# GreatV/oar-ocr

Measured on AMD Instinct MI355X. Metric: images/sec end-to-end PP-OCRv6 det+rec, higher is better.
Workload: dtype f32; 1 GPU; PP-OCRv6-tiny-class det+rec (synthetic-weight graphs: det 447089 params, rec 1135700 params, V=6906), batch=32 synthetic 960x960 pages per GPU, 40 text lines/page; timed region = u8 pages in pageable HOST memory -> oar_ocr_predict -> oar_ocr_decode -> sorted boxes + texts + scores on the host; image_batch_size=32, region_batch_size=256, parallelism=image-parallel x1

## Files before the change

### oar_ocr_amd/build.py

```python
from __future__ import annotations

import os
import subprocess
import sys
from concurrent.futures import ThreadPoolExecutor
from pathlib import Path

HERE = Path(__file__).resolve().parent
CSRC = HERE / "csrc"
LIBDIR = HERE / "lib"
LIB = LIBDIR / "libOarMi355x.so"
SOURCES = ["common.cc", "onnx_parse.cc", "engine.cc", "db_host.cc", "poly_host.cc", "pipeline.cc", "c_api.cc", "ctc_host.cc", "image_decode.cc", "image_misc_decode.cc", "jpeg_decode.cc", "layout.cc", "kernels.hip", "igemm.hip", "igemm_ws_1x1.hip", "igemm_ws_gen.hip", "igemm_ws_x6.hip", "igemm_os_x6.hip", "igemm_ws3.hip", "igemm_rs3_x6.hip", "prepost.hip", "contours.hip", "jpeg.hip", "layout.hip", "dsblock.hip", "dsblock_k3s1.hip", "dsblock_k3s2.hip", "dsblock_k5s1.hip", "dsblock_k5s2.hip", "dsblock_wa_a.hip", "dsblock_wa_b.hip", "dsblock_rs_k3s11.hip", "dsblock_rs_k3s21.hip", "dsblock_rs_k3s12.hip", "dsblock_rs_k3s22.hip", "dsblock_rs_dbg.hip", "dsblock_cs.hip", "dsblock_pc.hip", "dsblock_rs2.hip", "ctc_head_x6.hip", "chain.hip", "attention_x6.hip", "igemm_lk_x6.hip"]
HIPCC = os.environ.get("HIPCC", "/opt/rocm/bin/hipcc")
FLAGS = ["--offload-arch=gfx950", "-O3", "-std=c++17", "-fPIC", "-ffp-contract=off", "-fno-fast-math",
         "-Wno-unused-result", "-Wno-pass-failed"]
if os.environ.get("OAR_DSB_ABLATIONS"):
    FLAGS.append("-DOAR_DSB_ABLATIONS")


def _stale(out: Path, deps) -> bool:
    if not out.exists():
        return True
    t = out.stat().st_mtime
    return any(Path(d).stat().st_mtime > t for d in deps)


def build_lib(force: bool = False, verbose: bool = False) -> Path:
    LIBDIR.mkdir(exist_ok=True)
    objdir = LIBDIR / "obj"
    objdir.mkdir(exist_ok=True)
    headers = list(CSRC.glob("*.h")) + list(CSRC.glob("*.inc")) + [HERE.parent / "include" / "oar_mi355x.h"]
    jobs = []
    for s in SOURCES:
        src = CSRC / s
        obj = objdir / (s.replace(".", "_") + ".o")
        if force or _stale(obj, [src] + headers):
            jobs.append((src, obj))

    def cc(job):
        src, obj = job
        cmd = [HIPCC] + FLAGS + ["-c", str(src), "-o", str(obj)]
        if verbose:
            print(" ".join(cmd), flush=True)
        r = subprocess.run(cmd, capture_output=True, text=True)
        if r.returncode != 0:
            raise RuntimeError(f"hipcc failed for {src.name}:\n{r.stderr[-4000:]}")
        return obj

    if jobs:
        with ThreadPoolExecutor(max_workers=min(8, len(jobs))) as ex:
            list(ex.map(cc, jobs))
    objs = [objdir / (s.replace(".", "_") + ".o") for s in SOURCES]
    if force or jobs or _stale(LIB, objs):
        cmd = [HIPCC, "--offload-arch=gfx950", "-shared", "-fPIC", "-o", str(LIB)] + [str(o) for o in objs] + ["-lpthread", "-lz"]
        r = subprocess.run(cmd, capture_output=True, text=True)
        if r.returncode != 0:
            raise RuntimeError(f"link failed:\n{r.stderr[-4000:]}")
    return LIB


def csrc_fingerprint() -> str:
    import hashlib
    h = hashlib.sha256()
    for f in sorted(CSRC.iterdir()):
        if f.suffix in (".hip", ".inc", ".cc", ".h"):
            h.update(f.name.encode()); h.update(f.read_bytes())
    return h.hexdigest()[:16]


if __name__ == "__main__":
    p = build_lib(force="--force" in sys.argv, verbose=True)
    print(p, p.stat().st_size)
```

### oar_ocr_amd/csrc/engine.cc

```cpp
#include "engine.h"

#include "dsblock.h"

#include <algorithm>
#include <cmath>
#include <cstring>
#include <set>
#include <sstream>

namespace oar {

using k::Act;

static int64_t numel(const std::vector<int64_t>& d) {
    int64_t n = 1;
    for (auto v : d) n *= v;
    return n;
}

Engine::Engine(const uint8_t* onnx, size_t len, int device_id, hipStream_t caller_stream) : device_(device_id) {
    int ndev = 0;
    if (hipGetDeviceCount(&ndev) != hipSuccess || ndev <= 0)
        fail(OAR_DEVICE, "no HIP device visible: libOarMi355x has no CPU fallback");
    OAR_CHECK(device_id >= 0 && device_id < ndev, OAR_DEVICE, "device_id out of range");
// ... 502 lines not shown
        const char* fe = getenv("OAR_FUSE_SE_SCALE");
        const bool fuse = !fe || atoi(fe) != 0;
        auto cons = consumers(nodes);
        std::map<std::string, int> producer;
        for (int i = 0; i < (int)nodes.size(); ++i) for (auto& o : nodes[i].out) producer[o] = i;
        std::vector<bool> dead(nodes.size(), false);
        for (int i = 0; fuse && i < (int)nodes.size(); ++i) {
            const GNode& m = nodes[i];
            if (m.op != "Mul" || m.in.size() != 2 || m.act.kind != k::ACT_NONE || !m.residual.empty() || graph_outs.count(m.out[0])) continue;
            int gi = -1;
            for (int t = 0; t < 2; ++t) { auto pit = producer.find(m.in[t]); if (pit != producer.end() && nodes[pit->second].op == "SEGate") gi = t; }
            if (gi < 0 || cons[m.out[0]].size() != 1) continue;
            GNode& c = nodes[cons[m.out[0]][0]];
            if (c.op != "Conv" || c.in.size() < 2 || c.in.size() > 3 || c.in[0] != m.out[0] || !is_init(c.in[1]) || c.ai("group", 1) != 1) continue;
            const HostTensor& w = inits_[c.in[1]];
            if (w.dims.size() != 4 || w.dims[2] != 1 || w.dims[3] != 1) continue;
            bool plain = c.as("auto_pad", "NOTSET") == "NOTSET";
            for (auto v : c.ais("strides")) plain = plain && v == 1;
            for (auto v : c.ais("pads")) plain = plain && v == 0;
            if (!plain) continue;
            c.in.resize(4);
            c.in[0] = m.in[1 - gi];
            c.in[3] = m.in[gi];
            dead[i] = true;
        }
        std::vector<GNode> keep;
        for (int i = 0; i < (int)nodes.size(); ++i) if (!dead[i]) keep.push_back(std::move(nodes[i]));
        nodes.swap(keep);
    }
    {
        const char* fe = getenv("OAR_FUSE_SE_POOL");
        const bool fuse = !fe || atoi(fe) != 0;
        std::map<std::string, int> producer;
        for (int i = 0; i < (int)nodes.size(); ++i) for (auto& o : nodes[i].out) producer[o] = i;
        std::vector<bool> dead(nodes.size(), false);
        for (int i = 0; fuse && i < (int)nodes.size(); ++i) {
            const GNode& gp = nodes[i];
            if (gp.op != "GlobalAveragePool" || gp.in.size() != 1 || graph_outs.count(gp.out[0])) continue;
            auto pit = producer.find(gp.in[0]);
            if (pit == producer.end() || pit->second > i) continue;
            GNode& d = nodes[pit->second];
            if (d.op != "Conv" || d.out.size() != 1 || d.in.size() < 2 || d.in.size() > 3 || !is_init(d.in[1]) || !d.residual.empty()) continue;
            const HostTensor& wd = inits_[d.in[1]];
            if (wd.dims.size() != 4 || wd.dims[1] != 1 || d.ai("group", 1) != wd.dims[0] || wd.dims[0] < 8) continue;
            d.out.push_back(gp.out[0]);
            dead[i] = true;
            int readers = 0, gate = -1;
            for (int j = 0; j < (int)nodes.size(); ++j) {
                if (dead[j]) continue;
                for (size_t q = 0; q < nodes[j].in.size(); ++q) if (nodes[j].in[q] == gp.out[0]) { ++readers; if (nodes[j].op == "SEGate" && q == 0) gate = j; }
                if (nodes[j].residual == gp.out[0]) ++readers;
            }
            if (readers == 1 && gate >= 0 && !graph_outs.count(gp.out[0]) && !(fe && atoi(fe) == 1)) { Attr a; a.kind = Attr::I; a.i = 1; d.attrs["gap_raw"] = a; }
        }
        std::vector<GNode> keep;
        for (int i = 0; i < (int)nodes.size(); ++i) if (!dead[i]) keep.push_back(std::move(nodes[i]));
        nodes.swap(keep);
    }
    for (int i = 0; i < (int)nodes.size(); ++i) nodes[i].id = i;
    nodes_ = std::move(nodes);
}

struct TInfo {
    std::vector<int64_t> dims;
    Layout layout = Layout::NATIVE;
    Loc loc;
    bool host_int = false;
    std::vector<int64_t> hv;
    bool host_f = false;
    std::vector<double> hd;
    const HostTensor* ht = nullptr;
    bool is_int = false;
    bool u8_stem = false;
    std::string root;
    int gap_tiles = 0, gap_hw = 0;
    size_t bytes() const { return (size_t)std::max<int64_t>(numel(dims), 1) * 4; }
};

struct Arena {
    struct Blk { size_t off, sz; };
    std::vector<Blk> free_;
    size_t top = 0;
    static size_t al(size_t n) { return (n + 255) & ~(size_t)255; }
    size_t alloc(size_t n) {
        n = al(std::max<size_t>(n, 4));
        int best = -1;
        for (int i = 0; i < (int)free_.size(); ++i)
            if (free_[i].sz >= n && (best < 0 || free_[i].sz < free_[best].sz)) best = i;
        if (best >= 0) {
            size_t off = free_[best].off;
            if (free_[best].sz == n) free_.erase(free_.begin() + best);
            else { free_[best].off += n; free_[best].sz -= n; }
            return off;
        }
        size_t off = top;
        top += n;
        return off;
    }
    void release(size_t off, size_t n) {
        n = al(std::max<size_t>(n, 4));
        free_.push_back({off, n});
        std::sort(free_.begin(), free_.end(), [](const Blk& a, const Blk& b) { return a.off < b.off; });
        std::vector<Blk> m;
        for (auto& b : free_) {
            if (!m.empty() && m.back().off + m.back().sz == b.off) m.back().sz += b.sz;
            else m.push_back(b);
        }
        if (!m.empty() && m.back().off + m.back().sz == top) { top = m.back().off; m.pop_back(); }
        free_.swap(m);
    }
};

static std::vector<int64_t> clast_phys_dims(const std::vector<int64_t>& d) {
    std::vector<int64_t> p;
    p.push_back(d[0]);
    for (size_t i = 2; i < d.size(); ++i) p.push_back(d[i]);
    p.push_back(d[1]);
    return p;
}
static std::vector<int64_t> contig_strides(const std::vector<int64_t>& d) {
    std::vector<int64_t> s(d.size(), 1);
    for (int i = (int)d.size() - 2; i >= 0; --i) s[i] = s[i + 1] * d[i + 1];
    return s;
}

struct Planner {
    Engine& E;
    Plan& P;
    std::map<std::string, TInfo> vals;
    std::map<std::string, int> last_use;
    std::map<std::string, size_t> root_bytes;
    std::map<std::string, size_t> root_off;
    Arena arena;
    int cur = 0;
    std::vector<std::pair<size_t, size_t>> temps;

    Planner(Engine& e, Plan& p) : E(e), P(p) { opset = e.opset_; }

    struct PendingResize {
        Loc xin;
        std::vector<int64_t> dims;
        int N, H, W, C, Ho, Wo, imode, ictm, inm;
        float sh, sw;
        int fh = 0, fw = 0;
    };
    std::map<std::string, PendingResize> pending_resize;
    std::map<std::string, int> sole_consumer;
    void run_resize(const PendingResize& r, Loc yl, int64_t y_off, int y_ld) {
        const PendingResize q = r;
        step([=](const RunCtx& c) { k::resize(c.s, c.at(q.xin), c.mut(yl) + y_off, q.N, q.H, q.W, q.C, q.Ho, q.Wo, q.sh, q.sw, q.imode, q.ictm, q.inm, y_ld); }, 0,
             4.0 * ((double)q.N * q.H * q.W * q.C + (double)q.N * q.Ho * q.Wo * q.C));
    }
    std::map<std::string, const GNode*> pending_convt;
    struct PendingConcat { std::vector<Loc> src; std::vector<int> c; std::vector<int64_t> dims; };
    std::map<std::string, PendingConcat> pending_concat;
    std::map<std::string, int> concat_consumer;
    void emit_concat_gather(const PendingConcat& pc, Loc yl) {
        k::ConcatGatherP gp{};
        gp.n_src = (int)pc.src.size(); gp.N = (int)pc.dims[0]; gp.Ho = (int)pc.dims[2]; gp.Wo = (int)pc.dims[3]; gp.C = (int)pc.dims[1];
        int off = 0;
        for (size_t i = 0; i < pc.src.size(); ++i) { gp.c[i] = pc.c[i]; gp.off[i] = off; gp.fh[i] = 1; gp.fw[i] = 1; off += pc.c[i]; }
        const std::vector<Loc> src = pc.src;
        step([=](const RunCtx& c) {
            k::ConcatGatherP q = gp;
            for (int i = 0; i < q.n_src; ++i) q.x[i] = c.at(src[(size_t)i]);
            k::concat_gather(c.s, q, c.mut(yl));
        }, 0, 8.0 * (double)numel(pc.dims));
    }
    void materialise_concat(const std::string& name) {
        auto it = pending_concat.find(name);
        if (it == pending_concat.end()) return;
        const PendingConcat pc = it->second;
        pending_concat.erase(it);
        vals.erase(name);
        TInfo& y = new_out(name, pc.dims, Layout::CLAST);
        emit_concat_gather(pc, y.loc);
    }
    const PendingResize* peek_pending(const std::string& name) const {
        auto it = pending_resize.find(name);
        return it == pending_resize.end() ? nullptr : &it->second;
    }
    void materialise_pending(const std::string& name) {
        auto ct = pending_convt.find(name);
        if (ct != pending_convt.end()) {
            const GNode* node = ct->second;
            pending_convt.erase(ct);
            vals.erase(name);
            op_convt(*node, false);
            return;
        }
        auto it = pending_resize.find(name);
        if (it == pending_resize.end()) return;
        const PendingResize r = it->second;
        pending_resize.erase(it);
        TInfo& y = new_out(name, r.dims, Layout::CLAST);
        run_resize(r, y.loc, 0, r.C);
    }

    TInfo& get(const std::string& name) {
        if (!pending_resize.empty() || !pending_convt.empty()) materialise_pending(name);
        if (!pending_concat.empty()) materialise_concat(name);
        auto it = vals.find(name);
        if (it != vals.end()) return it->second;
        auto ii = E.inits_.find(name);
        OAR_CHECK(ii != E.inits_.end(), OAR_MODEL_LOAD, "graph references unknown value '" + name + "'");
        TInfo t;
        t.dims = ii->second.dims;
        if (ii->second.dtype == DType::F32) {
            t.ht = &ii->second;
            t.loc.kind = Loc::CONST;
            t.loc.cptr = E.upload_const("init:" + name, ii->second.f);
        } else {
            t.host_int = true;
            t.hv = ii->second.i;
        }
        return vals[name] = t;
    }
    bool has_input(const GNode& n, size_t i) const { return i < n.in.size() && !n.in[i].empty(); }

    Loc alloc_arena(size_t bytes, const std::string& root) {
        Loc l;
        l.kind = Loc::ARENA;
        l.off = (int64_t)arena.alloc(bytes);
        P.arena_bytes = std::max(P.arena_bytes, arena.top);
        if (!root.empty()) { root_bytes[root] = bytes; root_off[root] = (size_t)l.off; }
        return l;
    }
    Loc alloc_temp(size_t bytes) {
        Loc l = alloc_arena(bytes, "");
        temps.push_back({(size_t)l.off, bytes});
        return l;
    }
    std::map<std::string, std::vector<std::string>> root_aliases;
    TInfo& new_out(const std::string& name, const std::vector<int64_t>& dims, Layout lay) {
        TInfo t;
        t.dims = dims; t.layout = lay; t.root = name;
        t.loc = alloc_arena(t.bytes(), name);
        root_aliases[name].push_back(name);
        return vals[name] = t;
    }
    void adopt_root(const std::string& out, const std::string& tmp) {
        auto it = vals.find(out);
        if (it == vals.end() || tmp.empty() || tmp == out || it->second.root != tmp) return;
        auto rb = root_bytes.find(tmp);
        if (rb != root_bytes.end()) { root_bytes[out] = rb->second; root_off[out] = root_off[tmp]; root_bytes.erase(tmp); root_off.erase(tmp); }
        std::vector<std::string> moved;
        moved.swap(root_aliases[tmp]);
        root_aliases.erase(tmp);
        std::vector<std::string>& dst = root_aliases[out];
        for (auto& a : moved) {
            auto va = vals.find(a);
            if (va != vals.end() && va->second.root == tmp) { va->second.root = out; dst.push_back(a); }
        }
        it->second.root = out;
    }
    TInfo& alias_out(const std::string& name, const TInfo& src, const std::vector<int64_t>& dims, Layout lay, int64_t byte_off = 0) {
        TInfo t;
        t.dims = dims; t.layout = lay; t.root = src.root; t.loc = src.loc; t.ht = nullptr;
        if (t.loc.kind == Loc::CONST) t.loc.cptr = (const float*)((const char*)t.loc.cptr + byte_off);
        else t.loc.off += byte_off;
        if (!t.root.empty()) root_aliases[t.root].push_back(name);
        return vals[name] = t;
    }
    void step(std::function<void(const RunCtx&)> f, double flops = 0, double bytes = 0) {
        P.steps.push_back(std::move(f));
        P.flops += flops; P.bytes += bytes; P.n_kernels++;
        step_chain.push_back(-1);
        step_node.push_back(cur);
        static const bool dbg_steps = [] { const char* e = getenv("OAR_DEBUG_STEPS"); return e && atoi(e) != 0; }();
        if (dbg_steps) {
            const GNode* g = cur >= 0 && cur < (int)E.nodes_.size() ? &E.nodes_[(size_t)cur] : nullptr;
            P.step_ops.push_back(g ? g->op + " -> " + (g->out.empty() ? std::string("?") : g->out[0]) : std::string("?"));
        }
    }

    struct ChainRec {
        k::ChainOpD d;
        Loc in, out, res;
        int64_t rows = 0;
        int64_t fix_n = 0, fix_T = 0;
        std::function<std::vector<float>()> make_w;
        const float* dev_bias = nullptr;
        const float* dev_gamma = nullptr;
        double flops = 0, bytes = 0;
        int node = 0;
        std::string out_root;
    };
    std::vector<int> step_chain;
    std::vector<int> step_node;
    std::vector<ChainRec> chain_recs;
    bool chain_on = [] { const char* e = getenv("OAR_FUSE_CHAIN"); return !e || atoi(e) != 0; }();
    static bool chain_loc_ok(const Loc& l) { return l.kind == Loc::ARENA || l.kind == Loc::INPUT || (l.kind == Loc::CONST && l.cptr); }
    static k::ChainRef chain_ref(const Loc& l) {
        k::ChainRef r;
        if (l.kind == Loc::ARENA) { r.kind = 1; r.v = (unsigned long long)l.off; }
        else if (l.kind == Loc::INPUT) { r.kind = 2; r.v = (unsigned long long)l.off; }
        else if (l.kind == Loc::CONST) { r.kind = 0; r.v = (unsigned long long)reinterpret_cast<uintptr_t>(l.cptr); }
        return r;
    }
    void step_chainable(std::function<void(const RunCtx&)> f, ChainRec rec, double flops, double bytes) {
        step(std::move(f), flops, bytes);
        if (!chain_on) return;
        rec.flops = flops; rec.bytes = bytes; rec.node = cur;
        step_chain.back() = (int)chain_recs.size();
        chain_recs.push_back(std::move(rec));
    }
    bool chain_run_open() const { return chain_on && !step_chain.empty() && step_chain.back() >= 0; }
    static std::vector<float> chain_weight_conv(const HostTensor& W) {
        const int64_t Co = W.dims[0], Ci = W.dims[1], kw = W.dims[3], K = kw * Ci;
        std::vector<float> w((size_t)Co * K);
        for (int64_t co = 0; co < Co; ++co)
            for (int64_t ci = 0; ci < Ci; ++ci)
                for (int64_t b = 0; b < kw; ++b) w[(size_t)co * K + b * Ci + ci] = W.f[(size_t)((co * Ci + ci) * kw + b)];
        return w;
    }
    static std::vector<float> chain_weight_linear(const HostTensor& B, bool transB) {
        const int64_t K = transB ? B.dims[1] : B.dims[0], N = transB ? B.dims[0] : B.dims[1];
        std::vector<float> w((size_t)N * K);
        for (int64_t kk = 0; kk < K; ++kk)
            for (int64_t nn = 0; nn < N; ++nn) w[(size_t)nn * K + kk] = transB ? B.f[(size_t)(nn * K + kk)] : B.f[(size_t)(kk * N + nn)];
// ... 336 lines not shown
                float r1 = x - fh;
                std::memcpy(&um, &r1, 4); um &= 0xFFFF0000u;
                float fm; std::memcpy(&fm, &um, 4);
                float r2 = r1 - fm;
                std::memcpy(&ul, &r2, 4); ul &= 0xFFFF0000u;
                int64_t nf = r / 16, c = r % 16, kp = k / 32, half = (k % 32) / 16, g = (k % 16) / 4, e = half * 4 + k % 4;
                size_t lane = (size_t)(c + 16 * g);
                size_t base = (size_t)((nf * KP + kp) * 3) * 64 * 8;
                f[base + (0 * 64 + lane) * 8 + e] = (uint16_t)(uh >> 16);
                f[base + (1 * 64 + lane) * 8 + e] = (uint16_t)(um >> 16);
                f[base + (2 * 64 + lane) * 8 + e] = (uint16_t)(ul >> 16);
            }
        std::vector<float> out(f.size() / 2);
        std::memcpy(out.data(), f.data(), f.size() * 2);
        return out;
    }
    static std::vector<float> to_fragments(int fmt, const std::vector<float>& w, int64_t rows, int64_t K) {
        if (fmt == k::IGEMM_W_X6RS) return to_fragment_x6_rs(w, rows, K);
        return fmt == k::IGEMM_W_X6 ? to_fragment_x6(w, rows, K) : to_fragment_order(w, rows, K);
    }
    const float* conv_weight_igemm(const GNode& n, const HostTensor& W, int fmt) {
        std::string key = "igemm" + std::to_string(fmt) + ":" + n.in[1];
        auto it = E.dev_consts_.find(key);
        if (it != E.dev_consts_.end()) return it->second;
        int64_t Co = W.dims[0], Ci = W.dims[1], kh = W.dims[2], kw = W.dims[3];
        int64_t K = kh * kw * Ci, Cp = (Co + 63) / 64 * 64;
        std::vector<float> w((size_t)Cp * K, 0.f);
        for (int64_t co = 0; co < Co; ++co)
            for (int64_t ci = 0; ci < Ci; ++ci)
                for (int64_t a = 0; a < kh; ++a)
                    for (int64_t b = 0; b < kw; ++b)
                        w[(size_t)co * K + (a * kw + b) * Ci + ci] = W.f[((co * Ci + ci) * kh + a) * kw + b];
        (void)Cp;
        w.resize((size_t)Co * K);
        return E.upload_const(key, to_fragments(fmt, w, Co, K));
    }
    const float* conv_weight_cs(const GNode& dwn, const GNode& pwn, const HostTensor& WD, const HostTensor& WP, const std::vector<float>* bias_dw, const std::vector<float>* bias_pw) {
        std::string key = "dscs:" + dwn.in[1] + ":" + pwn.in[1];
        auto it = E.dev_consts_.find(key);
        if (it != E.dev_consts_.end()) return it->second;
        const int64_t C = WD.dims[0], ks = WD.dims[2], Co = WP.dims[0], nch = C / 16, nft = Co / 16;
        const size_t blk = k::dsblock_cs_block_bytes((int)ks, (int)nft), dwb = (size_t)(((ks * ks + 1) * 64 + 1023) / 1024 * 1024);
        std::vector<float> out(blk * (size_t)nch / 4 + (size_t)Co, 0.f);
        if (bias_pw) std::copy(bias_pw->begin(), bias_pw->begin() + Co, out.begin() + (ptrdiff_t)(blk * (size_t)nch / 4));
        auto split = [](float x, uint16_t& h, uint16_t& m, uint16_t& l) {
            uint32_t u, um, ul;
            std::memcpy(&u, &x, 4);
            const uint32_t uh = u & 0xFFFF0000u;
            float fh; std::memcpy(&fh, &uh, 4);
            const float r1 = x - fh;
            std::memcpy(&um, &r1, 4); um &= 0xFFFF0000u;
            float fm; std::memcpy(&fm, &um, 4);
            const float r2 = r1 - fm;
            std::memcpy(&ul, &r2, 4);
            h = (uint16_t)(uh >> 16); m = (uint16_t)(um >> 16); l = (uint16_t)(ul >> 16);
        };
        for (int64_t c = 0; c < nch; ++c) {
            char* b = reinterpret_cast<char*>(out.data()) + (size_t)c * blk;
            float* dw = reinterpret_cast<float*>(b);
            for (int64_t t = 0; t <= ks * ks; ++t)
                for (int64_t q = 0; q < 16; ++q) {
                    const int64_t ch = c * 16 + q;
                    dw[t * 16 + q] = t < ks * ks ? WD.f[(size_t)(ch * ks * ks + t)] : (bias_dw ? (*bias_dw)[(size_t)ch] : 0.f);
                }
            for (int64_t f = 0; f < nft; ++f) {
                uint16_t* lh = reinterpret_cast<uint16_t*>(b + dwb + (size_t)f * 1536);
                uint16_t* md = reinterpret_cast<uint16_t*>(b + dwb + (size_t)f * 1536 + 1024);
                for (int64_t g = 0; g < 4; ++g)
                    for (int64_t m = 0; m < 16; ++m)
                        for (int64_t e = 0; e < 4; ++e) {
                            uint16_t h, mm, l;
                            split(WP.f[(size_t)((f * 16 + m) * C + c * 16 + g * 4 + e)], h, mm, l);
                            const size_t lane = (size_t)(g * 16 + m);
                            lh[lane * 8 + e] = l; lh[lane * 8 + 4 + e] = h; md[lane * 4 + e] = mm;
                        }
            }
        }
        return E.upload_const(key, out);
    }
    const float* conv_weight_dw(const GNode& n, const HostTensor& W) {
        std::string key = "dw:" + n.in[1];
        auto it = E.dev_consts_.find(key);
        if (it != E.dev_consts_.end()) return it->second;
        int64_t C = W.dims[0], kh = W.dims[2], kw = W.dims[3];
        std::vector<float> w((size_t)C * kh * kw);
        for (int64_t c = 0; c < C; ++c)
            for (int64_t a = 0; a < kh; ++a)
                for (int64_t b = 0; b < kw; ++b) w[(size_t)(a * kw + b) * C + c] = W.f[(c * kh + a) * kw + b];
        return E.upload_const(key, w);
    }
    const float* conv_weight_direct(const GNode& n, const HostTensor& W) {
        std::string key = "direct:" + n.in[1];
        auto it = E.dev_consts_.find(key);
        if (it != E.dev_consts_.end()) return it->second;
        int64_t Co = W.dims[0], cpg = W.dims[1], kh = W.dims[2], kw = W.dims[3];
        std::vector<float> w((size_t)Co * cpg * kh * kw);
        for (int64_t co = 0; co < Co; ++co)
            for (int64_t ci = 0; ci < cpg; ++ci)
                for (int64_t a = 0; a < kh; ++a)
                    for (int64_t b = 0; b < kw; ++b)
                        w[(size_t)(((a * kw + b) * cpg + ci) * Co + co)] = W.f[((co * cpg + ci) * kh + a) * kw + b];
        return E.upload_const(key, w);
    }
    const float* convt_weight(const GNode& n, const HostTensor& W, bool igemm, int fmt = 0) {
        std::string key = (igemm ? "convt_ig" + std::to_string(fmt) + ":" : std::string("convt_dir:")) + n.in[1];
        auto it = E.dev_consts_.find(key);
        if (it != E.dev_consts_.end()) return it->second;
        int64_t Ci = W.dims[0], Co = W.dims[1], kh = W.dims[2], kw = W.dims[3];
        std::vector<float> w;
        if (igemm) {
            int64_t rows = kh * kw * Co;
            w.assign((size_t)rows * Ci, 0.f);
            for (int64_t ci = 0; ci < Ci; ++ci)
                for (int64_t co = 0; co < Co; ++co)
                    for (int64_t a = 0; a < kh; ++a)
                        for (int64_t b = 0; b < kw; ++b)
                            w[(size_t)((a * kw + b) * Co + co) * Ci + ci] = W.f[((ci * Co + co) * kh + a) * kw + b];
            w = to_fragments(fmt, w, rows, Ci);
        } else {
            w.assign((size_t)kh * kw * Ci * Co, 0.f);
            for (int64_t ci = 0; ci < Ci; ++ci)
                for (int64_t co = 0; co < Co; ++co)
                    for (int64_t a = 0; a < kh; ++a)
                        for (int64_t b = 0; b < kw; ++b)
                            w[(size_t)(((a * kw + b) * Ci + ci) * Co + co)] = W.f[((ci * Co + co) * kh + a) * kw + b];
        }
        return E.upload_const(key, w);
    }
    const float* linear_weight(const std::string& name, const HostTensor& B, bool transB, int fmt) {
        std::string key = "lin" + std::to_string(fmt) + ":" + (transB ? "t:" : "") + name;
        auto it = E.dev_consts_.find(key);
        if (it != E.dev_consts_.end()) return it->second;
        int64_t K = transB ? B.dims[1] : B.dims[0], N = transB ? B.dims[0] : B.dims[1];
        std::vector<float> w((size_t)N * K, 0.f);
        for (int64_t kk = 0; kk < K; ++kk)
            for (int64_t nn = 0; nn < N; ++nn) w[(size_t)nn * K + kk] = transB ? B.f[nn * K + kk] : B.f[kk * N + nn];
        return E.upload_const(key, to_fragments(fmt, w, N, K));
    }

    void get_pads(const GNode& n, int64_t H, int64_t W, int64_t kh, int64_t kw, int64_t sh, int64_t sw, int64_t dh, int64_t dw,
                  int64_t& pt, int64_t& pl, int64_t& pb, int64_t& pr) {
        std::vector<int64_t> pads = n.ais("pads");
        pt = pl = pb = pr = 0;
        if (pads.size() == 4) { pt = pads[0]; pl = pads[1]; pb = pads[2]; pr = pads[3]; }
        std::string ap = n.as("auto_pad", "NOTSET");
        if (ap == "SAME_UPPER" || ap == "SAME_LOWER") {
            int64_t oh = (H + sh - 1) / sh, ow = (W + sw - 1) / sw;
            int64_t th = std::max<int64_t>((oh - 1) * sh + (kh - 1) * dh + 1 - H, 0), tw = std::max<int64_t>((ow - 1) * sw + (kw - 1) * dw + 1 - W, 0);
            if (ap == "SAME_UPPER") { pt = th / 2; pb = th - pt; pl = tw / 2; pr = tw - pl; }
            else { pb = th / 2; pt = th - pb; pr = tw / 2; pl = tw - pr; }
        }
    }

    void op_conv(const GNode& n) {
        if (n.in.size() > 3 && !n.in[3].empty()) {
            TInfo xg = get(n.in[0]), gt = get(n.in[3]);
            const TInfo& wg = get(n.in[1]);
            bool ok = xg.dims.size() == 4 && !xg.host_int && !gt.host_int && wg.ht && wg.ht->dims.size() == 4 && gt.loc.kind != Loc::NONE && n.residual.empty();
            if (ok) {
                const int64_t N = xg.dims[0], C = xg.dims[1], HW = xg.dims[2] * xg.dims[3];
                ok = numel(gt.dims) == N * C && gt.dims.size() >= 2 && gt.dims[0] == N && gt.dims[1] == C && wg.ht->dims[1] == C && C % 8 == 0 &&
                     k::conv_igemm_se_ok(N * HW, (int)C, (int)wg.ht->dims[0], (int)HW);
            }
            if (!ok) {
                GNode mul;
                mul.op = "Mul"; mul.in = {n.in[0], n.in[3]}; mul.out = {n.out[0] + "::se"};
                op_binary(mul, 2);
                GNode c2 = n;
                c2.in.resize(3);
                c2.in[0] = mul.out[0];
                op_conv(c2);
                return;
            }
        }
        PendingConcat msrc;
        {
            auto pit = pending_concat.find(n.in[0]);
            if (pit != pending_concat.end()) {
                auto wi = E.inits_.find(n.in.size() > 1 ? n.in[1] : std::string());
                const std::vector<int64_t>& pd = pit->second.dims;
                const bool still_ok = wi != E.inits_.end() && wi->second.dims.size() == 4 && wi->second.dims[2] == 1 && wi->second.dims[3] == 1 && n.residual.empty() &&
                                      !(n.in.size() > 3 && !n.in[3].empty()) && n.out.size() == 1 &&
                                      k::conv_msrc_ok((long)(pd[0] * pd[2] * pd[3]), (int)pd[1], (int)wi->second.dims[0]);
                if (getenv("OAR_DEBUG_CONCAT")) fprintf(stderr, "  conv %s reads pending concat: still_ok=%d (w4=%d res=%d gate=%d nout=%zu)\n", n.out[0].c_str(), (int)still_ok, (int)(wi != E.inits_.end() && wi->second.dims.size() == 4), (int)!n.residual.empty(), (int)(n.in.size() > 3 && !n.in[3].empty()), n.out.size());
                if (still_ok) { msrc = pit->second; TInfo keep = vals[n.in[0]]; pending_concat.erase(pit); vals[n.in[0]] = keep; }
            }
        }
        TInfo x = get(n.in[0]);
        OAR_CHECK(x.dims.size() == 4, OAR_UNSUPPORTED_OP, "Conv: only 2-D convolutions are supported");
        const TInfo& wt = get(n.in[1]);
        OAR_CHECK(wt.ht, OAR_UNSUPPORTED_OP, "Conv: weights must be an initializer");
        const HostTensor& W = *wt.ht;
        OAR_CHECK(W.dims.size() == 4 && W.dims[0] > 0 && W.dims[1] > 0 && W.dims[2] > 0 && W.dims[3] > 0, OAR_MODEL_LOAD, "Conv: weight must be rank 4 with positive dims at " + n.out[0]);
        int64_t N = x.dims[0], Cin = x.dims[1], H = x.dims[2], Wd = x.dims[3];
        int64_t Cout = W.dims[0], kh = W.dims[2], kw = W.dims[3], g = n.ai("group", 1);
        OAR_CHECK(g >= 1 && W.dims[1] * g == Cin && Cout % g == 0, OAR_SHAPE_MISMATCH, "Conv: weight/input channel mismatch at " + n.out[0]);
        if (has_input(n, 2)) { const TInfo& bt = get(n.in[2]); OAR_CHECK(bt.ht && (int64_t)bt.ht->f.size() == Cout, OAR_MODEL_LOAD, "Conv: bias must be an f32 initializer of Cout elements at " + n.out[0]); }
        auto st = n.ais("strides"), dl = n.ais("dilations");
        int64_t sh = st.size() == 2 ? st[0] : 1, sw = st.size() == 2 ? st[1] : 1;
        int64_t dh = dl.size() == 2 ? dl[0] : 1, dw = dl.size() == 2 ? dl[1] : 1;
        int64_t pt, pl, pb, pr;
        get_pads(n, H, Wd, kh, kw, sh, sw, dh, dw, pt, pl, pb, pr);
        int64_t Ho = (H + pt + pb - dh * (kh - 1) - 1) / sh + 1, Wo = (Wd + pl + pr - dw * (kw - 1) - 1) / sw + 1;
        if (x.u8_stem) {
            OAR_CHECK(g == 1 && Cin == 3 && kh * kw * 3 <= 128 && n.residual.empty(), OAR_INTERNAL, "run_stem on a graph whose first node is not an RGB stem");
            const float* sb = has_input(n, 2) ? get(n.in[2]).loc.cptr : nullptr;
            TInfo& ys = new_out(n.out[0], {N, Cout, Ho, Wo}, Layout::CLAST);
            k::ConvP sp{};
            sp.N = (int)N; sp.H = (int)H; sp.W = (int)Wd; sp.Cin = 3; sp.Ho = (int)Ho; sp.Wo = (int)Wo; sp.Cout = (int)Cout;
            sp.kh = (int)kh; sp.kw = (int)kw; sp.sh = (int)sh; sp.sw = (int)sw; sp.pt = (int)pt; sp.pl = (int)pl; sp.dh = (int)dh; sp.dw = (int)dw;
            sp.groups = 1; sp.act = n.act; sp.bias = sb; sp.y_ld = (int)Cout; sp.convt2x2 = 0;
            sp.w = conv_weight_direct(n, W);
            const Loc ysl = ys.loc;
            step([=](const RunCtx& c) {
                OAR_CHECK(c.stem != nullptr, OAR_INTERNAL, "stem plan run without pages");
                k::ConvP q = sp;
                q.y = c.mut(ysl);
                k::conv_smallcin_u8(c.s, q, *c.stem);
            }, 2.0 * N * Ho * Wo * Cout * 3 * kh * kw, 3.0 * N * H * Wd + 4.0 * N * Ho * Wo * Cout);
            return;
        }
        Loc xin = msrc.src.empty() ? to_clast_loc(x) : Loc();
        const float* bias = has_input(n, 2) ? get(n.in[2]).loc.cptr : nullptr;
        Loc res;
        int res_up = 0;
        if (!n.residual.empty()) {
            const char* up_env = getenv("OAR_FUSE_RES_UP");
            const bool up_on = !up_env || atoi(up_env) != 0;
            if (const PendingResize* pr = peek_pending(n.residual)) {
                const bool f32_tile = g == 1 && Cin % 4 == 0 && Cout % 4 == 0 &&
                                      k::igemm_weight_format((long)(N * Ho * Wo), (int)(kh * kw * Cin), (int)Cout, kh == 1 && kw == 1 && sh == 1 && sw == 1 && pt == 0 && pl == 0, (int)Cin) == k::IGEMM_W_K16;
                if (up_on && f32_tile && pr->fh > 1 && pr->fh == pr->fw && pr->N == N && pr->C == Cout && pr->Ho == Ho && pr->Wo == Wo && Ho % pr->fh == 0 && Wo % pr->fw == 0 &&
                    pr->H * pr->fh == Ho && pr->W * pr->fw == Wo && N * Ho * Wo < ((int64_t)1 << 31)) {
                    res = pr->xin;
                    res_up = pr->fh;
                    pending_resize.erase(n.residual);
                }
            }
        }
        if (!n.residual.empty() && res_up == 0) {
            TInfo r = get(n.residual);
            if (r.host_int || r.dims != std::vector<int64_t>{N, Cout, Ho, Wo}) {
                GNode pre = n;
                pre.residual.clear();
                pre.out[0] = n.out[0] + "::pre";
                op_conv(pre);
                GNode add;
                add.op = "Add"; add.in = {pre.out[0], n.residual}; add.out = {n.out[0]};
                op_binary(add, 0);
                return;
            }
            res = to_clast_loc(r);
        }
        TInfo& y = new_out(n.out[0], {N, Cout, Ho, Wo}, Layout::CLAST);
        k::ConvP p{};
        p.N = (int)N; p.H = (int)H; p.W = (int)Wd; p.Cin = (int)Cin; p.Ho = (int)Ho; p.Wo = (int)Wo; p.Cout = (int)Cout;
        p.kh = (int)kh; p.kw = (int)kw; p.sh = (int)sh; p.sw = (int)sw; p.pt = (int)pt; p.pl = (int)pl; p.dh = (int)dh; p.dw = (int)dw;
        p.groups = (int)g; p.act = n.act; p.bias = bias; p.y_ld = (int)Cout; p.convt2x2 = 0; p.res_up = res_up;
        int kind;
        const int64_t cg = Cin / g, og = Cout / g;
        const char* gx_env = getenv("OAR_GROUPED_X6");
        const bool grouped_x6 = g > 1 && g < Cin && cg % 8 == 0 && og % 4 == 0 && !(n.in.size() > 3 && !n.in[3].empty()) && res_up == 0 && !(gx_env && gx_env[0] == '0') &&
                                k::conv_grouped_x6_ok((long)(N * Ho * Wo), (int)(kh * kw * cg), (int)og, (int)cg);
        std::vector<const float*> wgrp;
        std::vector<int> slices3;
        if (grouped_x6) {
            kind = 3;
            p.w_fmt = k::IGEMM_W_X6;
            const size_t per = (size_t)(og * cg * kh * kw);
            for (int64_t gi = 0; gi < g; ++gi) {
                HostTensor Wg;
                Wg.dtype = DType::F32; Wg.dims = {og, cg, kh, kw};
                Wg.f.assign(W.f.begin() + (ptrdiff_t)(gi * per), W.f.begin() + (ptrdiff_t)((gi + 1) * per));
                GNode gn = n;
                gn.in[1] = n.in[1] + "::group" + std::to_string(gi);
                wgrp.push_back(conv_weight_igemm(gn, Wg, k::IGEMM_W_X6));
            }
        }
        else if (g == 1 && Cout <= 16 && Cin > 64 && kh == 3 && kw == 3 && sh == 1 && sw == 1 && pt == 1 && pl == 1 && dh == 1 && dw == 1 && Ho == H && Wo == Wd && n.residual.empty() &&
                 !(n.in.size() > 3 && !n.in[3].empty()) && !(slices3 = k::conv3x3_n16_slices((long)(N * Ho * Wo), (int)Cin, (int)Cout, (long)(H * Wd), (int)(4 * Cout))).empty()) {
            kind = 4;
            p.w_fmt = k::IGEMM_W_X6;
            int64_t c0 = 0;
            for (int cs : slices3) {
                HostTensor Ws;
                Ws.dtype = DType::F32; Ws.dims = {Cout, (int64_t)cs, kh, kw};
                Ws.f.resize((size_t)(Cout * cs * 9));
                for (int64_t co = 0; co < Cout; ++co)
                    for (int64_t ci = 0; ci < cs; ++ci)
                        for (int64_t t = 0; t < 9; ++t) Ws.f[(size_t)((co * cs + ci) * 9 + t)] = W.f[(size_t)((co * Cin + c0 + ci) * 9 + t)];
                GNode gn = n;
                gn.in[1] = n.in[1] + "::slice" + std::to_string(c0);
                wgrp.push_back(conv_weight_igemm(gn, Ws, k::IGEMM_W_X6));
                c0 += cs;
            }
        }
        else if (g == 1 && Cin % 4 == 0) {
            kind = 0;
            const bool is1x1 = kh == 1 && kw == 1 && sh == 1 && sw == 1 && pt == 0 && pl == 0;
            const bool same3x3 = kh == 3 && kw == 3 && sh == 1 && sw == 1 && pt == 1 && pl == 1 && dh == 1 && dw == 1 && Ho == H && Wo == Wd && n.residual.empty();
            const bool lk_ok = !(n.in.size() > 3 && !n.in[3].empty()) && res_up == 0 &&
                               k::conv_lk_x6_eligible((int)kh, (int)kw, (int)sh, (int)sw, (int)pt, (int)pl, (int)dh, (int)dw, (int)H, (int)Wd, (int)Ho, (int)Wo, (int)Cin, (int)Cout, (int)(4 * Cout), (long)(N * Ho * Wo));
            p.w_fmt = k::igemm_weight_format((long)(N * Ho * Wo), (int)(kh * kw * Cin), (int)Cout, is1x1, (int)Cin, same3x3 ? (long)(H * Wd) : 0, lk_ok);
            p.w = conv_weight_igemm(n, W, p.w_fmt);
        }
        else if (g == Cin && g == Cout && Cout % 4 == 0) { kind = 1; p.w = conv_weight_dw(n, W); }
        else { kind = 2; p.w = conv_weight_direct(n, W); }
        Loc yl = y.loc;
        bool has_res = res.kind != Loc::NONE;
        Loc gate;
        if (n.in.size() > 3 && !n.in[3].empty()) {
            OAR_CHECK(kind == 0 && (p.w_fmt == k::IGEMM_W_X6 || p.w_fmt == k::IGEMM_W_K16), OAR_INTERNAL, "Conv: gate on a layer that is on neither gated kernel");
            gate = get(n.in[3]).loc;
        }
        const bool has_gate = gate.kind != Loc::NONE;
        double flops = 2.0 * N * Ho * Wo * Cout * (Cin / g) * kh * kw;
        double bytes = 4.0 * (N * H * Wd * Cin + N * Ho * Wo * Cout * (has_res ? 2 : 1) + numel(W.dims));
        if (n.out.size() > 1) {
            const int tiles = kind == 1 ? k::conv_dw_gap_tiles(p) : 0;
            if (tiles > 0 && Cout <= 1024 && n.ai("gap_raw", 0) != 0) {
                TInfo& gy = new_out(n.out[1], {N, (int64_t)tiles * Cout, 1, 1}, Layout::CLAST);
                gy.gap_tiles = tiles; gy.gap_hw = (int)(Ho * Wo);
                const Loc part = gy.loc;
                step([=](const RunCtx& c) {
                    k::ConvP q = p;
                    q.x = c.at(xin); q.y = c.mut(yl); q.residual = has_res ? c.at(res) : nullptr; q.gap_part = c.mut(part);
                    k::conv_dw(c.s, q);
                }, flops, bytes + 4.0 * N * tiles * Cout);
                return;
            }
            if (tiles > 0 && Cout <= 1024) {
                TInfo& gy = new_out(n.out[1], {N, Cout, 1, 1}, Layout::CLAST);
                const Loc gl = gy.loc, part = alloc_temp((size_t)N * tiles * Cout * sizeof(float));
                const int hw = (int)(Ho * Wo);
                step([=](const RunCtx& c) {
                    k::ConvP q = p;
                    q.x = c.at(xin); q.y = c.mut(yl); q.residual = has_res ? c.at(res) : nullptr; q.gap_part = c.mut(part);
                    k::conv_dw(c.s, q);
                }, flops, bytes + 4.0 * N * tiles * Cout);
                step([=](const RunCtx& c) { k::global_avgpool_finish(c.s, c.at(part), c.mut(gl), (int)N, tiles, (int)Cout, hw); }, 0, 4.0 * N * tiles * Cout);
                return;
            }
        }
        const bool from_concat = !msrc.src.empty();
        OAR_CHECK(!from_concat || (kind == 0 && p.w_fmt == k::IGEMM_W_X6), OAR_INTERNAL, "Conv: deferred concat in front of a layer that is not on the bf16x6 kernels");
        auto run = [=](const RunCtx& c) {
            k::ConvP q = p;
            q.y = c.mut(yl); q.residual = has_res ? c.at(res) : nullptr; q.se = has_gate ? c.at(gate) : nullptr;
            if (from_concat) {
                q.x = nullptr; q.n_msrc = (int)msrc.src.size();
                for (int i = 0; i < q.n_msrc; ++i) { q.msrc[i] = c.at(msrc.src[(size_t)i]); q.msrc_c[i] = msrc.c[(size_t)i]; }
            } else {
                q.x = c.at(xin);
            }
            if (kind == 3) {
                const int ng = p.groups, cgi = p.Cin / ng, ogi = p.Cout / ng;
                for (int gi = 0; gi < ng; ++gi) {
                    k::ConvP r = q;
                    r.groups = 1; r.Cin = cgi; r.Cout = ogi; r.x_ld = p.Cin;
                    r.x = q.x + (size_t)gi * cgi; r.y = q.y + (size_t)gi * ogi; r.w = wgrp[(size_t)gi];
                    r.bias = q.bias ? q.bias + (size_t)gi * ogi : nullptr;
                    r.residual = q.residual ? q.residual + (size_t)gi * ogi : nullptr;
                    k::conv_igemm(c.s, r);
                }
                return;
            }
            if (kind == 4) {
                int c0 = 0;
                for (size_t i = 0; i < slices3.size(); ++i) {
                    k::ConvP r = q;
                    r.Cin = slices3[i]; r.x_ld = p.Cin; r.x = q.x + c0; r.w = wgrp[i]; r.accum = i > 0 ? 1 : 0;
                    if (i > 0) r.bias = nullptr;
                    if (i + 1 < slices3.size()) r.act = k::Act{};
                    k::conv_igemm(c.s, r);
                    c0 += slices3[i];
                }
                return;
            }
            if (kind == 0) k::conv_igemm(c.s, q);
            else if (kind == 1) k::conv_dw(c.s, q);
            else k::conv_direct(c.s, q);
        };
        auto pool_after = [&]() {
            if (n.out.size() < 2) return;
            GNode gp;
            gp.op = "GlobalAveragePool"; gp.in = {n.out[0]}; gp.out = {n.out[1]};
            op_gap(gp);
        };
        if (kind == 0 && !has_gate && H == 1 && Ho == 1 && kh == 1 && pt == 0 && pb == 0 && sw == 1 && dw == 1 && Wo == Wd && Cin % 16 == 0 && Cout % 16 == 0 && k::chain_act_ok(n.act.kind) &&
            chain_loc_ok(xin) && (!has_res || chain_loc_ok(res))) {
            ChainRec r;
            r.d.type = k::CH_GEMM; r.d.K = (int)(kw * Cin); r.d.N = (int)Cout; r.d.cin = (int)Cin; r.d.pad = (int)pl;
            r.d.in_ld = (int)Cin; r.d.out_ld = (int)Cout; r.d.res_ld = (int)Cout;
            r.d.act = n.act.kind; r.d.alpha = n.act.alpha; r.d.beta = n.act.beta; r.dev_bias = bias;
            r.in = xin; r.out = yl; if (has_res) r.res = res;
            r.rows = N * Wd; r.out_root = n.out[0];
            if (kw > 1) { r.fix_n = N; r.fix_T = Wd; }
            const HostTensor* Wp = &W;
            r.make_w = [Wp]() { return chain_weight_conv(*Wp); };
            step_chainable(run, std::move(r), flops, bytes);
            pool_after();
            return;
        }
        step(run, flops, bytes);
        pool_after();
    }

    bool dsblock_shape(const GNode& n, int64_t N, int64_t C, int64_t H, int64_t W, k::DsBlockP& p) {
        const TInfo &wdt = get(n.in[1]), &wpt = get(n.in[3]);
        if (!wdt.ht || !wpt.ht) return false;
        const HostTensor &WD = *wdt.ht, &WP = *wpt.ht;
        const int64_t ks = WD.dims[2], Cout = WP.dims[0];
        if (WD.dims[0] != C || WP.dims[1] != C) return false;
        auto st = n.ais("strides");
        const int64_t sh = st.size() == 2 ? st[0] : 1, sw = st.size() == 2 ? st[1] : 1;
        int64_t pt, pl, pb, pr;
        get_pads(n, H, W, ks, ks, sh, sw, 1, 1, pt, pl, pb, pr);
        const int64_t Ho = (H + pt + pb - (ks - 1) - 1) / sh + 1, Wo = (W + pl + pr - (ks - 1) - 1) / sw + 1;
        p = k::DsBlockP{};
        p.N = (int)N; p.H = (int)H; p.W = (int)W; p.C = (int)C; p.Ho = (int)Ho; p.Wo = (int)Wo; p.Cout = (int)Cout;
        p.ks = (int)ks; p.sh = (int)sh; p.sw = (int)sw; p.pt = (int)pt; p.pl = (int)pl;
        p.act1.kind = (int)n.ai("act1", 0); p.act1.alpha = n.af("act1_alpha", 0.f); p.act1.beta = n.af("act1_beta", 0.f);
        p.act2 = n.act; p.y_ld = (int)Cout;
        p.has_res = !n.residual.empty();
        return Ho > 0 && Wo > 0;
    }
    bool dsblock_link_ok(int i) {
        if (i + 1 >= (int)E.nodes_.size()) return false;
        const GNode &n = E.nodes_[i], &m = E.nodes_[i + 1];
        if (n.op != "DSBlock" || m.op != "DSBlock" || !n.residual.empty() || !m.residual.empty() || m.in.empty() || m.in[0] != n.out[0]) return false;
        for (auto& o : E.output_names_) if (o == n.out[0]) return false;
        for (int j = 0; j < (int)E.nodes_.size(); ++j) {
            if (j == i + 1) continue;
            const GNode& q = E.nodes_[j];
            for (auto& s : q.in) if (s == n.out[0]) return false;
            if (q.residual == n.out[0]) return false;
        }
        for (size_t k = 1; k < m.in.size(); ++k) if (m.in[k] == n.out[0]) return false;
        return true;
    }
    std::map<int, bool> dsblock_pair_plan;
    void plan_dsblock_run(int first, const TInfo& x) {
        std::vector<k::DsBlockP> ps;
        std::vector<bool> link;
        int64_t N = x.dims[0], C = x.dims[1], H = x.dims[2], W = x.dims[3];
        for (int i = first; i < (int)E.nodes_.size(); ++i) {
            const GNode& q = E.nodes_[i];
            k::DsBlockP p;
            if (q.op != "DSBlock" || q.in.size() < 5 || !dsblock_shape(q, N, C, H, W, p)) break;
            ps.push_back(p);
            C = p.Cout; H = p.Ho; W = p.Wo;
            const bool ok = dsblock_link_ok(i);
            link.push_back(ok);
            if (!ok) break;
        }
        const int R = (int)ps.size();
        std::vector<double> w(std::max(R - 1, 0), -1.0);
        for (int j = 0; j + 1 < R; ++j)
            if (link[j] && k::dsblock2_eligible(ps[j], ps[j + 1])) w[j] = (double)N * ps[j].Cout * ps[j].Ho * ps[j].Wo;
        static const bool greedy_first = [] { const char* e = getenv("OAR_DSBLOCK_RS2_FIRST"); return e && atoi(e) != 0; }();
        std::vector<bool> take(std::max(R - 1, 0), false);
        if (greedy_first) {
            for (int j = 0; j + 1 < R; ++j) if (w[j] > 0) { take[j] = true; ++j; }
        } else {
            std::vector<double> best(R + 1, 0.0);
            for (int j = R - 2; j >= 0; --j) best[j] = std::max(best[j + 1], w[j] > 0 ? w[j] + best[std::min(j + 2, R)] : 0.0);
            for (int j = 0; j + 1 < R;) {
                if (w[j] > 0 && w[j] + best[std::min(j + 2, R)] >= best[j + 1]) { take[j] = true; j += 2; }
                else ++j;
            }
        }
        for (int j = 0; j < R; ++j) dsblock_pair_plan[first + j] = j + 1 < R && take[j];
    }
    bool try_dsblock_pair(const GNode& n, const TInfo& x) {
        if (cur + 1 >= (int)E.nodes_.size() || !n.residual.empty() || x.dims.size() != 4 || x.host_int) return false;
        if (!dsblock_pair_plan.count(cur)) plan_dsblock_run(cur, x);
        if (!dsblock_pair_plan[cur]) return false;
        const GNode& m = E.nodes_[cur + 1];
        k::DsBlockP pa, pb;
        const int64_t N = x.dims[0], C = x.dims[1], H = x.dims[2], W = x.dims[3];
        if (!dsblock_shape(n, N, C, H, W, pa) || !dsblock_shape(m, N, pa.Cout, pa.Ho, pa.Wo, pb) || !k::dsblock2_eligible(pa, pb)) return false;
        auto weights = [&](const GNode& d, k::DsBlockP& p) {
            const HostTensor &WD = *get(d.in[1]).ht, &WP = *get(d.in[3]).ht;
            GNode dwn, pwn;
            dwn.op = "Conv"; dwn.in = {d.in[0], d.in[1]};
            pwn.op = "Conv"; pwn.in = {d.out[0] + "::dw", d.in[3]};
            if (!d.in[2].empty()) OAR_CHECK((int64_t)get(d.in[2]).ht->f.size() == p.C, OAR_MODEL_LOAD, "DSBlock: depthwise bias size");
            if (!d.in[4].empty()) OAR_CHECK((int64_t)get(d.in[4]).ht->f.size() == p.Cout, OAR_MODEL_LOAD, "DSBlock: pointwise bias size");
            p.wd = conv_weight_dw(dwn, WD);
            p.bd = d.in[2].empty() ? nullptr : get(d.in[2]).loc.cptr;
            p.wp = conv_weight_igemm(pwn, WP, k::IGEMM_W_X6RS);
            p.bp = d.in[4].empty() ? nullptr : get(d.in[4]).loc.cptr;
        };
        weights(n, pa);
        weights(m, pb);
        Loc xin = to_clast_loc(x);
        TInfo& y = new_out(m.out[0], {N, (int64_t)pb.Cout, (int64_t)pb.Ho, (int64_t)pb.Wo}, Layout::CLAST);
        Loc yl = y.loc;
        const double px = (double)N * H * W;
        const double flops = 2.0 * px * (pa.C * (9.0 + pa.Cout) + pb.C * (9.0 + pb.Cout));
        const double bytes = 4.0 * px * (pa.C + pb.Cout);
        step([=](const RunCtx& c) {
            k::DsBlockP qa = pa, qb = pb;
            qa.x = c.at(xin); qb.y = c.mut(yl);
// ... 691 lines not shown
        Loc xin = x.loc;
        TInfo& y = new_out(n.out[0], od, clast ? Layout::CLAST : Layout::NATIVE);
        Loc yl = y.loc;
        step([=](const RunCtx& c) { k::pad_nd(c.s, c.at(xin), c.mut(yl), r, pin.data(), pout.data(), pbef.data(), imode, value); }, 0, 8.0 * numel(od));
    }

    void op_gap(const GNode& n) {
        TInfo x = get(n.in[0]);
        OAR_CHECK(x.dims.size() == 4, OAR_UNSUPPORTED_OP, "GlobalAveragePool: rank-4 only");
        Loc xin = to_clast_loc(x);
        int64_t N = x.dims[0], C = x.dims[1], HW = x.dims[2] * x.dims[3];
        TInfo& y = new_out(n.out[0], {N, C, 1, 1}, Layout::CLAST);
        Loc yl = y.loc;
        const int splits = k::global_avgpool_splits((int)N, (int)HW, (int)C);
        Loc part;
        if (splits > 1) part = alloc_temp((size_t)N * splits * C * sizeof(float));
        step([=](const RunCtx& c) { k::global_avgpool(c.s, c.at(xin), c.mut(yl), (int)N, (int)HW, (int)C, splits > 1 ? c.mut(part) : nullptr); }, 0, 4.0 * numel(x.dims));
    }

    void op_pool(const GNode& n, bool is_max) {
        TInfo x = get(n.in[0]);
        OAR_CHECK(x.dims.size() == 4, OAR_UNSUPPORTED_OP, "Pool: rank-4 only");
        auto ks = n.ais("kernel_shape"), st = n.ais("strides");
        OAR_CHECK(ks.size() == 2, OAR_UNSUPPORTED_OP, "Pool: kernel_shape");
        int64_t kh = ks[0], kw = ks[1], sh = st.size() == 2 ? st[0] : 1, sw = st.size() == 2 ? st[1] : 1;
        int64_t pt, pl, pb, pr;
        get_pads(n, x.dims[2], x.dims[3], kh, kw, sh, sw, 1, 1, pt, pl, pb, pr);
        bool ceil_mode = n.ai("ceil_mode", 0) != 0;
        auto od = [&](int64_t in, int64_t k_, int64_t s_, int64_t p0, int64_t p1) {
            int64_t t = in + p0 + p1 - k_;
            int64_t o = (ceil_mode ? (t + s_ - 1) / s_ : t / s_) + 1;
            if (ceil_mode && (o - 1) * s_ >= in + p0) --o;
            return o;
        };
        int64_t Ho = od(x.dims[2], kh, sh, pt, pb), Wo = od(x.dims[3], kw, sw, pl, pr);
        Loc xin = to_clast_loc(x);
        TInfo& y = new_out(n.out[0], {x.dims[0], x.dims[1], Ho, Wo}, Layout::CLAST);
        k::PoolP p{};
        p.N = (int)x.dims[0]; p.H = (int)x.dims[2]; p.W = (int)x.dims[3]; p.C = (int)x.dims[1]; p.Ho = (int)Ho; p.Wo = (int)Wo;
        p.kh = (int)kh; p.kw = (int)kw; p.sh = (int)sh; p.sw = (int)sw; p.pt = (int)pt; p.pl = (int)pl; p.pb = (int)pb; p.pr = (int)pr;
        p.is_max = is_max; p.count_include_pad = (int)n.ai("count_include_pad", 0);
        Loc yl = y.loc;
        auto run = [=](const RunCtx& c) { k::PoolP q = p; q.x = c.at(xin); q.y = c.mut(yl); k::pool2d(c.s, q); };
        const double bytes = 4.0 * (numel(x.dims) + numel(y.dims));
        const char* cpe = getenv("OAR_CHAIN_POOL");
        if (!(cpe && cpe[0] == '0') && !is_max && !ceil_mode && Ho == 1 && kh == x.dims[2] && kw == sw && kw * Wo <= x.dims[3] && x.dims[3] - kw * Wo < kw && pt == 0 && pl == 0 && pb == 0 && pr == 0 &&
            (p.C & 3) == 0 && kh * kw <= 64 && chain_loc_ok(xin)) {
            ChainRec r;
            r.d.type = k::CH_POOL; r.d.K = (int)kh; r.d.cin = (int)kw; r.d.pad = (int)x.dims[3]; r.d.N = p.C; r.d.in_ld = p.C; r.d.out_ld = p.C;
            r.in = xin; r.out = yl; r.rows = x.dims[0] * Wo; r.fix_n = x.dims[0]; r.fix_T = Wo; r.out_root = n.out[0];
            step_chainable(run, std::move(r), 0, bytes);
        } else {
            step(run, 0, bytes);
        }
    }

    void op_resize(const GNode& n) {
        TInfo x = get(n.in[0]);
        OAR_CHECK(x.dims.size() == 4, OAR_UNSUPPORTED_OP, "Resize: rank-4 only");
        int64_t H = x.dims[2], W = x.dims[3], Ho, Wo;
        float sh, sw;
        if (has_input(n, 3)) {
            const TInfo& sz = get(n.in[3]);
            OAR_CHECK(sz.host_int && sz.hv.size() == 4, OAR_UNSUPPORTED_OP, "Resize: sizes must be a host int tensor");
            Ho = sz.hv[2]; Wo = sz.hv[3]; sh = (float)Ho / (float)H; sw = (float)Wo / (float)W;
        } else {
            OAR_CHECK(has_input(n, 2), OAR_UNSUPPORTED_OP, "Resize: neither scales nor sizes");
            const TInfo& sc = get(n.in[2]);
            std::vector<double> scv = host_values(sc);
            OAR_CHECK(host_evaluable(sc) && scv.size() == 4, OAR_UNSUPPORTED_OP, "Resize: scales must be 4 floats known at plan time");
            sh = (float)scv[2]; sw = (float)scv[3];
            Ho = (int64_t)std::floor((float)H * sh); Wo = (int64_t)std::floor((float)W * sw);
        }
        std::string mode = n.as("mode", "nearest"), ctm = n.as("coordinate_transformation_mode", "half_pixel"), nm = n.as("nearest_mode", "round_prefer_floor");
        int imode = mode == "nearest" ? 0 : 1;
        OAR_CHECK(mode == "nearest" || mode == "linear", OAR_UNSUPPORTED_OP, "Resize: mode " + mode);
        int ictm = ctm == "asymmetric" ? 0 : ctm == "half_pixel" ? 1 : ctm == "align_corners" ? 2 : ctm == "pytorch_half_pixel" ? 3 : -1;
        OAR_CHECK(ictm >= 0, OAR_UNSUPPORTED_OP, "Resize: coordinate_transformation_mode " + ctm);
        int inm = nm == "floor" ? 0 : nm == "round_prefer_floor" ? 1 : nm == "round_prefer_ceil" ? 2 : 3;
        static const bool defer_on = [] { const char* e = getenv("OAR_DEFER_RESIZE"); return !e || atoi(e) != 0; }();
        if (defer_on && imode == 0 && x.layout == Layout::CLAST && sole_consumer.count(n.out[0])) {
            PendingResize r;
            r.xin = x.loc; r.dims = {x.dims[0], x.dims[1], Ho, Wo};
            r.N = (int)x.dims[0]; r.H = (int)H; r.W = (int)W; r.C = (int)x.dims[1]; r.Ho = (int)Ho; r.Wo = (int)Wo;
            r.imode = imode; r.ictm = ictm; r.inm = inm; r.sh = sh; r.sw = sw;
            auto factor = [&](int in, int out, float scale) {
                if (in <= 0 || out % in != 0) return 0;
                const int f = out / in;
                for (int o = 0; o < out; ++o) if (k::resize_nearest_index(o, scale, in, out, ictm, inm) != o / f) return 0;
                return f;
            };
            r.fh = factor(r.H, r.Ho, sh); r.fw = factor(r.W, r.Wo, sw);
            if (!r.fh || !r.fw) r.fh = r.fw = 0;
            pending_resize[n.out[0]] = r;
            TInfo t;
            t.dims = r.dims; t.layout = Layout::CLAST; t.root = "";
            vals[n.out[0]] = t;
            return;
        }
        Loc xin = to_clast_loc(x);
        TInfo& y = new_out(n.out[0], {x.dims[0], x.dims[1], Ho, Wo}, Layout::CLAST);
        Loc yl = y.loc;
        int N = (int)x.dims[0], C = (int)x.dims[1];
        step([=](const RunCtx& c) { k::resize(c.s, c.at(xin), c.mut(yl), N, (int)H, (int)W, C, (int)Ho, (int)Wo, sh, sw, imode, ictm, inm, C); }, 0,
             4.0 * (numel(x.dims) + numel(y.dims)));
    }

    void op_concat(const GNode& n) {
        bool absorb = false;
        if (!pending_resize.empty()) {
            int64_t axis0 = n.ai("axis", 0);
            bool ok = true, any = false;
            int64_t total_c = 0;
            for (auto& s : n.in) {
                const PendingResize* pr = peek_pending(s);
                any = any || pr;
                auto it = vals.find(s);
                if (it == vals.end() || it->second.dims.size() != 4 || it->second.layout != Layout::CLAST || it->second.host_int) { ok = false; break; }
                if ((it->second.dims[1] & 3) != 0) ok = false;
                total_c += it->second.dims[1];
            }
            absorb = any && ok && (axis0 == 1 || axis0 == -3) && (total_c & 3) == 0;
            if (!absorb) for (auto& s : n.in) materialise_pending(s);
        }
        std::vector<TInfo> xs;
        for (auto& s : n.in) { auto it = vals.find(s); xs.push_back(absorb && peek_pending(s) ? it->second : get(s)); }
        bool all_host = true, any_host = false, any_f = false;
        for (auto& t : xs) { all_host = all_host && host_evaluable(t) && t.dims.size() <= 1; any_host = any_host || t.host_int; any_f = any_f || float_like(t); }
        if (all_host && any_host) {
            std::vector<double> v;
            for (auto& t : xs) { std::vector<double> e = host_values(t); v.insert(v.end(), e.begin(), e.end()); }
            set_host(n.out[0], {(int64_t)v.size()}, v, any_f);
            return;
        }
        int r = (int)xs[0].dims.size();
        int64_t axis = n.ai("axis", 0);
        if (axis < 0) axis += r;
        bool clast = false;
        for (auto& t : xs) clast = clast || (t.layout == Layout::CLAST);
        std::vector<int64_t> od = xs[0].dims;
        od[axis] = 0;
        for (auto& t : xs) od[axis] += t.dims[axis];
        if (clast && r >= 3) {
            int pax = axis == 0 ? 0 : (axis == 1 ? r - 1 : (int)axis - 1);
            std::vector<int64_t> pod = clast_phys_dims(od);
            int64_t outer = 1, inner = 1;
            for (int i = 0; i < pax; ++i) outer *= pod[i];
            for (int i = pax + 1; i < r; ++i) inner *= pod[i];
            std::vector<Loc> ins;
            for (size_t i = 0; i < xs.size(); ++i) ins.push_back(absorb && peek_pending(n.in[i]) ? Loc() : to_clast_loc(xs[i]));
            int64_t coff = 0, total = pod[pax] * inner;
            bool plain = !absorb && r == 4 && inner == 1 && xs.size() >= 3 && (od[1] & 3) == 0;
            for (auto& t : xs) plain = plain && t.dims.size() == 4 && (t.dims[1] & 3) == 0;
            static const bool defer_on = [] { const char* e = getenv("OAR_CONCAT_DEFER"); return !(e && e[0] == '0'); }();
            if (getenv("OAR_DEBUG_CONCAT")) fprintf(stderr, "concat %s: plain=%d absorb=%d r=%d inner=%ld n=%zu consumer=%d\n", n.out[0].c_str(), (int)plain, (int)absorb, r, (long)inner, xs.size(), concat_consumer.count(n.out[0]) ? concat_consumer[n.out[0]] : -1);
            if (plain && defer_on && xs.size() <= 8 && concat_consumer.count(n.out[0])) {
                const GNode& cn = E.nodes_[concat_consumer[n.out[0]]];
                auto wi = E.inits_.find(cn.in.size() > 1 ? cn.in[1] : std::string());
                auto attr_ok = [&](const char* a, int64_t want) { auto v = cn.ais(a); for (auto e : v) if (e != want) return false; return true; };
                bool ok = wi != E.inits_.end() && wi->second.dims.size() == 4 && wi->second.dims[2] == 1 && wi->second.dims[3] == 1 && wi->second.dims[1] == od[1] && cn.ai("group", 1) == 1 &&
                          attr_ok("strides", 1) && attr_ok("pads", 0) && attr_ok("dilations", 1) && cn.residual.empty() && !(cn.in.size() > 3 && !cn.in[3].empty()) &&
                          cn.as("auto_pad", "NOTSET") == "NOTSET";
                for (auto& t : xs) ok = ok && t.layout == Layout::CLAST && (t.dims[1] & 7) == 0 && t.dims[0] == od[0] && t.dims[2] == od[2] && t.dims[3] == od[3] && !t.host_int;
                if (getenv("OAR_DEBUG_CONCAT")) {
                    fprintf(stderr, "  ok before msrc check = %d (K=%ld N=%ld) res=%d gate=%d autopad=%s\n", (int)ok, (long)od[1], wi != E.inits_.end() ? (long)wi->second.dims[0] : -1L, (int)!cn.residual.empty(), (int)(cn.in.size() > 3 && !cn.in[3].empty()), cn.as("auto_pad", "NOTSET").c_str());
                    for (auto& t : xs) fprintf(stderr, "    src layout=%d C=%ld host=%d\n", (int)(t.layout == Layout::CLAST), (long)t.dims[1], (int)t.host_int);
                }
                ok = ok && k::conv_msrc_ok((long)(od[0] * od[2] * od[3]), (int)od[1], (int)wi->second.dims[0]) && (wi->second.dims[0] & 3) == 0;
                if (ok) {
                    PendingConcat pc;
                    for (size_t i = 0; i < xs.size(); ++i) { pc.src.push_back(ins[i]); pc.c.push_back((int)xs[i].dims[1]); }
                    pc.dims = od;
                    TInfo t;
                    t.dims = od; t.layout = Layout::CLAST;
                    vals[n.out[0]] = t;
                    pending_concat[n.out[0]] = std::move(pc);
                    return;
                }
            }
            TInfo& y = new_out(n.out[0], od, Layout::CLAST);
            Loc yl = y.loc;
            if ((absorb || plain) && r == 4 && inner == 1 && xs.size() <= 8) {
                static const bool gather_on = [] { const char* e = getenv("OAR_CONCAT_GATHER"); return !(e && e[0] == '0'); }();
                bool ok = gather_on;
                for (size_t i = 0; ok && i < xs.size(); ++i) {
                    const PendingResize* pr = peek_pending(n.in[i]);
                    if (pr) ok = pr->fh > 0 && pr->fw > 0 && pr->imode == 0 && pr->Ho == od[2] && pr->Wo == od[3] && pr->H * pr->fh == pr->Ho && pr->W * pr->fw == pr->Wo && pr->N == od[0];
                    else ok = xs[i].dims[0] == od[0] && xs[i].dims[2] == od[2] && xs[i].dims[3] == od[3];
                }
                if (ok) {
                    k::ConcatGatherP gp{};
                    std::vector<Loc> src(xs.size());
                    gp.n_src = (int)xs.size(); gp.N = (int)od[0]; gp.Ho = (int)od[2]; gp.Wo = (int)od[3]; gp.C = (int)od[1];
                    double bytes = 4.0 * (double)numel(od);
                    for (size_t i = 0; i < xs.size(); ++i) {
                        const PendingResize* pr = peek_pending(n.in[i]);
                        src[i] = pr ? pr->xin : ins[i];
                        gp.c[i] = (int)xs[i].dims[1]; gp.off[i] = (int)coff; gp.fh[i] = pr ? pr->fh : 1; gp.fw[i] = pr ? pr->fw : 1;
                        bytes += 4.0 * (double)numel(xs[i].dims) / (gp.fh[i] * gp.fw[i]);
                        coff += xs[i].dims[1];
                    }
                    for (auto& nm : n.in) pending_resize.erase(nm);
                    step([=](const RunCtx& c) {
                        k::ConcatGatherP q = gp;
                        for (int i = 0; i < q.n_src; ++i) q.x[i] = c.at(src[(size_t)i]);
                        k::concat_gather(c.s, q, c.mut(yl));
                    }, 0, bytes);
                    return;
                }
            }
            for (size_t i = 0; i < xs.size(); ++i) {
                int64_t w = xs[i].dims[axis] * inner;
                Loc il = ins[i];
                int64_t off = coff;
                if (absorb && peek_pending(n.in[i])) {
                    run_resize(*peek_pending(n.in[i]), yl, off, (int)total);
                    pending_resize.erase(n.in[i]);
                } else {
                    concat_copy_step(il, yl, off, outer, w, total, n.out[0]);
                }
                coff += w;
            }
            return;
        }
        int64_t outer = 1, inner = 1;
        for (int i = 0; i < axis; ++i) outer *= od[i];
        for (int i = (int)axis + 1; i < r; ++i) inner *= od[i];
        std::vector<Loc> ins;
        for (auto& t : xs) ins.push_back(to_native_loc(t));
        TInfo& y = new_out(n.out[0], od, Layout::NATIVE);
        Loc yl = y.loc;
        int64_t coff = 0, total = od[axis] * inner;
        for (size_t i = 0; i < xs.size(); ++i) {
            int64_t w = xs[i].dims[axis] * inner;
            Loc il = ins[i];
            int64_t off = coff;
            concat_copy_step(il, yl, off, outer, w, total, n.out[0]);
            coff += w;
        }
    }
    void concat_copy_step(Loc il, Loc yl, int64_t off, int64_t outer, int64_t w, int64_t total, const std::string& out_name) {
        auto run = [=](const RunCtx& c) { k::copy2d(c.s, c.at(il), c.mut(yl) + off, outer, (int)w, (int)w, (int)total); };
        if ((w & 3) == 0 && (total & 3) == 0 && (off & 3) == 0 && chain_loc_ok(il) && yl.kind == Loc::ARENA) {
            ChainRec r;
            r.d.type = k::CH_COPY; r.d.N = (int)w; r.d.in_ld = (int)w; r.d.out_ld = (int)total;
            r.in = il; r.out = yl; r.out.off += off * 4; r.rows = outer; r.out_root = out_name;
            step_chainable(run, std::move(r), 0, 8.0 * outer * w);
        } else {
            step(run, 0, 8.0 * outer * w);
        }
    }

    void view_native(const GNode& n, const TInfo& x, const std::vector<int64_t>& od) {
        OAR_CHECK(numel(od) == numel(x.dims), OAR_SHAPE_MISMATCH, "reshape: element count mismatch at " + n.out[0]);
        if (x.layout == Layout::CLAST) {
            int r = (int)x.dims.size();
            int64_t sp = 1;
            for (int i = 2; i < r; ++i) sp *= x.dims[i];
            if (od.size() >= 3 && od[0] == x.dims[0] && od[1] == x.dims[1] && !x.ht) { alias_out(n.out[0], x, od, Layout::CLAST); return; }
            if (x.dims[1] != 1 && sp != 1) {
                TInfo& y = new_out(n.out[0], od, Layout::NATIVE);
                to_native_loc(x, y.loc);
                return;
            }
        }
        alias_out(n.out[0], x, od, Layout::NATIVE);
    }

    void op_reshape(const GNode& n) {
        TInfo x = get(n.in[0]);
        const TInfo& sh = get(n.in[1]);
        OAR_CHECK(sh.host_int, OAR_UNSUPPORTED_OP, "Reshape: shape must be known on the host");
        if (x.host_int) { TInfo o = x; o.dims.assign(sh.hv.begin(), sh.hv.end()); vals[n.out[0]] = o; return; }
        std::vector<int64_t> od(sh.hv.size());
        int64_t known = 1; int infer = -1;
        for (size_t i = 0; i < od.size(); ++i) {
            int64_t v = sh.hv[i];
            if (v == 0 && n.ai("allowzero", 0) == 0) v = x.dims[i];
            if (v == -1) { infer = (int)i; v = 1; }
            od[i] = v; known *= v;
        }
        if (infer >= 0) od[infer] = numel(x.dims) / std::max<int64_t>(known, 1);
        view_native(n, x, od);
    }

    void op_flatten(const GNode& n) {
        TInfo x = get(n.in[0]);
        int64_t ax = n.ai("axis", 1);
        if (ax < 0) ax += (int64_t)x.dims.size();
        int64_t a = 1, b = 1;
        for (int i = 0; i < (int)x.dims.size(); ++i) (i < ax ? a : b) *= x.dims[i];
        view_native(n, x, {a, b});
    }

    std::vector<int64_t> axes_of(const GNode& n, size_t input_idx) {
        if (has_input(n, input_idx)) { const TInfo& a = get(n.in[input_idx]); OAR_CHECK(a.host_int, OAR_UNSUPPORTED_OP, "axes must be host ints"); return a.hv; }
        return n.ais("axes");
    }

    void op_squeeze(const GNode& n) {
        TInfo x = get(n.in[0]);
        std::vector<int64_t> axes = axes_of(n, 1);
        int r = (int)x.dims.size();
        std::set<int> ax;
        if (axes.empty()) { for (int i = 0; i < r; ++i) if (x.dims[i] == 1) ax.insert(i); }
        for (auto a : axes) ax.insert((int)(a < 0 ? a + r : a));
        std::vector<int64_t> od;
        for (int i = 0; i < r; ++i) if (!ax.count(i)) od.push_back(x.dims[i]);
        if (x.host_int) { TInfo o = x; o.dims = od; vals[n.out[0]] = o; return; }
        if (x.layout == Layout::CLAST && !ax.count(0) && !ax.count(1) && od.size() >= 3) { alias_out(n.out[0], x, od, Layout::CLAST); return; }
        view_native(n, x, od);
    }

    void op_unsqueeze(const GNode& n) {
        TInfo x = get(n.in[0]);
        std::vector<int64_t> axes = axes_of(n, 1);
        int r = (int)x.dims.size() + (int)axes.size();
        std::set<int> ax;
        for (auto a : axes) ax.insert((int)(a < 0 ? a + r : a));
        std::vector<int64_t> od;
        size_t j = 0;
        for (int i = 0; i < r; ++i) od.push_back(ax.count(i) ? 1 : x.dims[j++]);
        if (x.host_int) { TInfo o = x; o.dims = od; vals[n.out[0]] = o; return; }
        if (x.layout == Layout::CLAST && !ax.count(0) && !ax.count(1) && r <= 5) { alias_out(n.out[0], x, od, Layout::CLAST); return; }
// ... 223 lines not shown
        TInfo& y = new_out(n.out[0], od, Layout::NATIVE);
        Loc yl = y.loc;
        k::GemmP g{};
        g.batch = (int)batch; g.M = (int)M; g.N = (int)N; g.K = (int)K; g.transB = 0; g.alpha = 1.0f;
        g.sA = na == 1 ? 0 : M * K; g.sB = nb == 1 ? 0 : K * N; g.sC = M * N; g.act = n.act;
        step([=](const RunCtx& c) { k::GemmP q = g; q.A = c.at(al); q.B = c.at(bl); q.C = c.mut(yl); k::gemm_batched(c.s, q); },
             2.0 * batch * M * N * K, 4.0 * batch * (M * K + K * N + M * N));
    }

    void op_softmax(const GNode& n) {
        TInfo x = get(n.in[0]);
        int r = (int)x.dims.size();
        int64_t axis = n.ai("axis", E_opset13() ? -1 : 1);
        if (axis < 0) axis += r;
        Loc xin = to_native_loc(x);
        int64_t C, rows;
        if (E_opset13() && axis != r - 1 && !x.host_int) {
            std::vector<int64_t> perm;
            for (int i = 0; i < r; ++i) if (i != axis) perm.push_back(i);
            perm.push_back(axis);
            std::vector<int64_t> inv(r);
            for (int i = 0; i < r; ++i) inv[perm[i]] = i;
            GNode t1; t1.op = "Transpose"; t1.in = {n.in[0]}; t1.out = {n.out[0] + "::moved"};
            Attr p1; p1.kind = Attr::IS; p1.is = perm; t1.attrs["perm"] = p1;
            op_transpose(t1);
            GNode sm = n; sm.in = {t1.out[0]}; sm.out = {n.out[0] + "::sm"};
            Attr la; la.kind = Attr::I; la.i = -1; sm.attrs["axis"] = la;
            op_softmax(sm);
            GNode t2; t2.op = "Transpose"; t2.in = {sm.out[0]}; t2.out = {n.out[0]};
            Attr p2; p2.kind = Attr::IS; p2.is = inv; t2.attrs["perm"] = p2;
            op_transpose(t2);
            adopt_root(n.out[0], sm.out[0]);
            return;
        }
        if (E_opset13()) {
            OAR_CHECK(axis == r - 1, OAR_UNSUPPORTED_OP, "Softmax: only the last axis is supported");
            C = x.dims.back(); rows = numel(x.dims) / std::max<int64_t>(C, 1);
        } else {
            rows = 1; C = 1;
            for (int i = 0; i < r; ++i) (i < axis ? rows : C) *= x.dims[i];
        }
        TInfo& y = new_out(n.out[0], x.dims, Layout::NATIVE);
        Loc yl = y.loc;
        step([=](const RunCtx& c) { k::softmax_lastdim(c.s, c.at(xin), c.mut(yl), rows, (int)C); }, 4.0 * rows * C, 8.0 * rows * C);
    }
    void op_attention(const GNode& n) {
        TInfo x = get(n.in[0]);
        const int64_t h = n.ai("heads", 1), d = n.ai("head_dim", 1);
        OAR_CHECK(x.dims.size() == 3 && x.dims[2] == 3 * h * d, OAR_SHAPE_MISMATCH, "Attention: input must be [n, T, 3*heads*head_dim]");
        const int64_t N = x.dims[0], T = x.dims[1];
        OAR_CHECK(k::attention_fits((int)T, (int)h, (int)d), OAR_UNSUPPORTED_OP, "Attention: head_dim must be in 1..=64");
        Loc xin = to_native_loc(x);
        TInfo& y = new_out(n.out[0], {N, T, h * d}, Layout::NATIVE);
        Loc yl = y.loc;
        const float scale = n.af("scale", 1.0f);
        auto run = [=](const RunCtx& c) { k::attention(c.s, c.at(xin), c.mut(yl), (int)N, (int)T, (int)h, (int)d, scale); };
        const double flops = 4.0 * N * h * T * T * d, bytes = 4.0 * N * T * 4 * h * d;
        if (d <= k::kChainMaxHd && d % 4 == 0 && chain_loc_ok(xin)) {
            ChainRec r;
            r.d.type = k::CH_ATTN; r.d.heads = (int)h; r.d.hd = (int)d; r.d.scale = scale; r.d.N = (int)(h * d);
            r.d.in_ld = (int)(3 * h * d); r.d.out_ld = (int)(h * d);
            r.in = xin; r.out = yl; r.rows = N * T; r.fix_n = N; r.fix_T = T; r.out_root = n.out[0];
            step_chainable(run, std::move(r), flops, bytes);
        } else {
            step(run, flops, bytes);
        }
    }
    bool E_opset13() const { return opset >= 13 || opset == 0; }
    int64_t opset = 17;

    void op_layernorm(const GNode& n) {
        TInfo x = get(n.in[0]);
        int r = (int)x.dims.size();
        int64_t axis = n.ai("axis", -1);
        if (axis < 0) axis += r;
        OAR_CHECK(axis == r - 1, OAR_UNSUPPORTED_OP, "LayerNormalization: only the last axis is supported");
        Loc xin = to_native_loc(x);
        const float* g = has_input(n, 1) ? get(n.in[1]).loc.cptr : nullptr;
        const float* b = has_input(n, 2) ? get(n.in[2]).loc.cptr : nullptr;
        int64_t C = x.dims.back(), rows = numel(x.dims) / std::max<int64_t>(C, 1);
        float eps = n.af("epsilon", 1e-5f);
        TInfo& y = new_out(n.out[0], x.dims, Layout::NATIVE);
        Loc yl = y.loc;
        auto run = [=](const RunCtx& c) { k::layernorm(c.s, c.at(xin), g, b, c.mut(yl), rows, (int)C, eps); };
        if (chain_loc_ok(xin) && C > 0) {
            ChainRec r;
            r.d.type = k::CH_LN; r.d.N = (int)C; r.d.in_ld = (int)C; r.d.out_ld = (int)C; r.d.eps = eps; r.dev_gamma = g; r.dev_bias = b;
            r.in = xin; r.out = yl; r.rows = rows; r.out_root = n.out[0];
            step_chainable(run, std::move(r), 8.0 * rows * C, 8.0 * rows * C);
        } else {
            step(run, 8.0 * rows * C, 8.0 * rows * C);
        }
    }

    void op_host_arith(const GNode& n, int op) {
        const TInfo &a = get(n.in[0]), &b = get(n.in[1]);
        TInfo o; o.host_int = true;
        size_t cnt = std::max(a.hv.size(), b.hv.size());
        for (size_t i = 0; i < cnt; ++i) {
            int64_t x = a.hv[a.hv.size() == 1 ? 0 : i], y = b.hv[b.hv.size() == 1 ? 0 : i], v = 0;
            switch (op) { case 0: v = x + y; break; case 1: v = x - y; break; case 2: v = x * y; break; default: v = y ? x / y : 0; }
            o.hv.push_back(v);
        }
        o.dims = a.hv.size() >= b.hv.size() ? a.dims : b.dims;
        vals[n.out[0]] = o;
    }

    void compute_last_use() {
        static const std::set<std::string> alias_ops = {"Reshape", "Flatten", "Squeeze", "Unsqueeze", "Transpose", "Identity", "Split", "Slice", "Gather", "Cast"};
        std::map<std::string, int> lu;
        for (int i = 0; i < (int)E.nodes_.size(); ++i) {
            const GNode& n = E.nodes_[i];
            for (auto& s : n.in) if (!s.empty()) lu[s] = i;
            if (!n.residual.empty()) lu[n.residual] = i;
        }
        for (auto& o : E.output_names_) lu[o] = 1 << 30;
        sole_consumer.clear();
        {
            std::map<std::string, std::pair<int, int>> uses;
            for (int i = 0; i < (int)E.nodes_.size(); ++i) {
                const GNode& n = E.nodes_[i];
                for (auto& s : n.in) if (!s.empty()) { auto& u = uses[s]; ++u.first; u.second = i; }
                if (!n.residual.empty()) { auto& u = uses[n.residual]; ++u.first; u.second = i; }
            }
            for (int i = 0; i < (int)E.nodes_.size(); ++i) {
                const GNode& n = E.nodes_[i];
                if ((n.op != "Resize" && n.op != "ConvTranspose") || n.out.empty() || n.in.empty()) continue;
                auto u = uses.find(n.out[0]);
                if (u == uses.end() || u->second.first != 1) continue;
                if (std::find(E.output_names_.begin(), E.output_names_.end(), n.out[0]) != E.output_names_.end()) continue;
                sole_consumer[n.out[0]] = u->second.second;
                int& l = lu[n.in[0]];
                l = std::max(l, u->second.second);
            }
        }
        concat_consumer.clear();
        {
            std::map<std::string, std::pair<int, int>> uses;
            for (int i = 0; i < (int)E.nodes_.size(); ++i) {
                const GNode& n = E.nodes_[i];
                for (auto& s : n.in) if (!s.empty()) { auto& u = uses[s]; ++u.first; u.second = i; }
                if (!n.residual.empty()) { auto& u = uses[n.residual]; ++u.first; u.second = i; }
            }
            for (int i = 0; i < (int)E.nodes_.size(); ++i) {
                const GNode& n = E.nodes_[i];
                if (n.op != "Concat" || n.out.empty() || n.in.size() < 3) continue;
                auto u = uses.find(n.out[0]);
                if (u == uses.end() || u->second.first != 1) continue;
                if (std::find(E.output_names_.begin(), E.output_names_.end(), n.out[0]) != E.output_names_.end()) continue;
                const GNode& cn = E.nodes_[u->second.second];
                if (cn.op != "Conv" || cn.in.empty() || cn.in[0] != n.out[0]) continue;
                concat_consumer[n.out[0]] = u->second.second;
                for (auto& sname : n.in) { int& l = lu[sname]; l = std::max(l, u->second.second); }
            }
        }
        for (int i = (int)E.nodes_.size() - 1; i >= 0; --i) {
            const GNode& n = E.nodes_[i];
            if (!alias_ops.count(n.op) || n.in.empty()) continue;
            int m = lu.count(n.in[0]) ? lu[n.in[0]] : i;
            for (auto& o : n.out) if (lu.count(o)) m = std::max(m, lu[o]);
            lu[n.in[0]] = m;
        }
        last_use = lu;
    }

    int read_after(const std::string& v) const { auto it = last_use.find(v); return it == last_use.end() ? -1 : it->second; }
    std::string node_desc(int i) const {
        const GNode& g = E.nodes_[(size_t)i];
        return "node " + std::to_string(i) + " (" + g.op + " -> " + (g.out.empty() ? std::string("?") : g.out[0]) + ")";
    }
    int checked_upto = -1;
    void check_release(const std::vector<std::string>& dead, int i) {
        for (auto& d : dead) {
            auto al = root_aliases.find(d);
            if (al == root_aliases.end()) continue;
            for (auto& v : al->second) {
                auto vi = vals.find(v);
                if (vi == vals.end() || vi->second.root != d || vi->second.loc.kind != Loc::ARENA) continue;
                const int r = read_after(v);
                OAR_CHECK(r <= i, OAR_INTERNAL, "plan liveness: " + node_desc(i) + " frees root '" + d + "' but '" + v + "' lives in it and is read " +
                          (r >= (1 << 30) ? std::string("as a graph output") : "at node " + std::to_string(r)));
            }
        }
        for (int j = checked_upto + 1; j <= i; ++j) {
            for (auto& o : E.nodes_[(size_t)j].out) {
                auto vi = vals.find(o);
                if (vi == vals.end() || vi->second.loc.kind != Loc::ARENA || read_after(o) <= i) continue;
                const std::string& rt = vi->second.root;
                OAR_CHECK(!rt.empty() && root_bytes.count(rt), OAR_INTERNAL, "plan liveness: '" + o + "' of " + node_desc(j) + " is read after " + node_desc(i) +
                          (rt.empty() ? std::string(" but lives in a per-node temp") : " but its root '" + rt + "' is not booked"));
            }
        }
        checked_upto = i;
    }
    void release_dead(int i) {
        for (auto& t : temps) arena.release(t.first, t.second);
        temps.clear();
        std::vector<std::string> dead;
        for (auto& rb : root_bytes) {
            auto it = last_use.find(rb.first);
            int lu = it == last_use.end() ? i : it->second;
            if (lu <= i) dead.push_back(rb.first);
        }
        for (auto& d : dead) { arena.release(root_off[d], root_bytes[d]); root_bytes.erase(d); root_off.erase(d); }
        check_release(dead, i);
        for (auto& d : dead) root_aliases.erase(d);
    }

    bool skip_final_softmax = false;
    std::set<int> fused_into_prev;
    bool stem_u8 = false;
    void build(const std::vector<int64_t>& in_dims, bool in_clast, const std::vector<std::vector<int64_t>>* extra_dims) {
        compute_last_use();
        TInfo in;
        in.u8_stem = stem_u8;
        in.dims = in_dims;
        in.layout = (in_clast && in_dims.size() >= 3) ? Layout::CLAST : Layout::NATIVE;
        in.loc.kind = Loc::INPUT;
        in.root = "";
        vals[E.input_name_] = in;
        for (size_t i = 1; extra_dims && i < extra_dims->size() && i < E.input_infos_.size(); ++i) {
            TInfo ex;
            ex.dims = (*extra_dims)[i];
            ex.layout = Layout::NATIVE;
            ex.loc.kind = Loc::EXTRA;
            ex.loc.idx = (int)i;
            ex.root = "";
            vals[E.input_infos_[i].name] = ex;
        }
        for (int i = 0; i < (int)E.nodes_.size(); ++i) {
            const GNode& n = E.nodes_[i];
            cur = i;
            if (fused_into_prev.count(i)) { release_dead(i); continue; }
            if (skip_final_softmax && n.op == "Softmax" && !n.out.empty() && n.out[0] == E.output_names_[0]) {
                TInfo x = get(n.in[0]);
                int r = (int)x.dims.size();
                int64_t axis = n.ai("axis", -1);
                if (axis < 0) axis += r;
                if (E_opset13() && axis == r - 1 && x.layout == Layout::NATIVE) {
                    alias_out(n.out[0], x, x.dims, Layout::NATIVE);
                    adopt_root(n.out[0], x.root);
                    P.skipped_softmax = true;
                    release_dead(i);
                    continue;
                }
            }
            dispatch(n);
            if (!chain_run_open()) release_dead(i);
        }
        for (size_t oi = 0; oi < E.output_names_.size(); ++oi) {
            const std::string& on = E.output_names_[oi];
            auto it = vals.find(on);
            OAR_CHECK(it != vals.end(), OAR_MODEL_LOAD, "graph output '" + on + "' was never produced");
            TInfo t = it->second;
            PlanOutput po;
            po.name = on; po.dims = t.dims;
            const int declared = oi < E.output_infos_.size() ? E.output_infos_[oi].elem_type : 0;
            if (t.host_int) {
                po.on_host = true;
                po.dtype = t.host_f ? 1 : 7;
                if (t.host_f) po.host_vals = t.hd;
                else po.host_vals.assign(t.hv.begin(), t.hv.end());
                OAR_CHECK((int64_t)po.host_vals.size() == numel(t.dims), OAR_INTERNAL, "host output '" + on + "': value / shape mismatch");
                P.outputs.push_back(po);
                continue;
            }
            po.dtype = (t.is_int || declared == 7 || declared == 6) ? 7 : 1;
            OAR_CHECK(t.loc.kind != Loc::ARENA || (!t.root.empty() && root_bytes.count(t.root)), OAR_INTERNAL,
                      "plan liveness: graph output '" + on + "' lives in " + (t.root.empty() ? std::string("a per-node temp") : "root '" + t.root + "', which was released"));
            if (t.layout == Layout::CLAST) { po.has_clast = true; po.loc_clast = t.loc; }
            Loc nat = to_native_loc(t);
            if (nat.kind == Loc::ARENA && nat.off != t.loc.off) {
                for (auto it2 = temps.begin(); it2 != temps.end(); ++it2)
                    if ((int64_t)it2->first == nat.off) { temps.erase(it2); break; }
            }
            po.loc = nat;
            P.outputs.push_back(po);
        }
        P.arena_bytes = std::max<size_t>(P.arena_bytes, 256);
        fuse_chains();
    }

    void dispatch(const GNode& n) {
        const std::string& op = n.op;
        auto info = [&](const std::string& s) -> const TInfo& { return (peek_pending(s) || pending_convt.count(s) || pending_concat.count(s)) ? vals.find(s)->second : get(s); };
        bool host_inputs = !n.in.empty();
        for (auto& s : n.in) if (!s.empty()) host_inputs = host_inputs && info(s).host_int;
        if (op == "Shape") {
            const TInfo& x = get(n.in[0]);
            TInfo o; o.host_int = true; o.hv = x.dims; o.dims = {(int64_t)x.dims.size()};
            vals[n.out[0]] = o; return;
        }
        bool evaluable = !n.in.empty(), any_host = false;
        for (auto& s : n.in) if (!s.empty()) { const TInfo& t = info(s); evaluable = evaluable && host_evaluable(t); any_host = any_host || t.host_int; }
        if (evaluable && (any_host || op == "Range") && op_host(n)) return;
        (void)host_inputs;
        if (op == "ConstantOfShape") return op_constant_of_shape(n);
        if (op == "Conv") return op_conv(n);
        if (op == "ConvTranspose") return op_convt(n);
        if (op == "BatchNormalization") return op_bn(n);
        if (is_unary_act(op)) return op_unary(n, act_of(n));
        if (op == "Clip") {
            Act a; a.kind = k::ACT_CLIP; a.alpha = n.af("min", -3.402823466e38f); a.beta = n.af("max", 3.402823466e38f);
            if (has_input(n, 1)) { const TInfo& t = get(n.in[1]); OAR_CHECK(t.ht, OAR_UNSUPPORTED_OP, "Clip: dynamic min"); a.alpha = t.ht->f[0]; }
            if (has_input(n, 2)) { const TInfo& t = get(n.in[2]); OAR_CHECK(t.ht, OAR_UNSUPPORTED_OP, "Clip: dynamic max"); a.beta = t.ht->f[0]; }
            return op_unary(n, a);
// ... 282 lines not shown
```

### oar_ocr_amd/csrc/igemm.hip

```cpp
#include "igemm_dev.h"

namespace oar {
namespace k {

template <int NT, int PF, bool IS1X1>
__global__ __launch_bounds__(256, 2) void conv_igemm_kernel(IgemmP p) {
    const int lane = threadIdx.x & 63, wave = threadIdx.x >> 6;
    const int pl_ = lane & 15, g = lane >> 4;
    const long b = blockIdx.x;
    const int xcd = (int)(b & 7);
    const long slot = b >> 3;
    const int ntile = (int)(slot % p.ny);
    const long mtile = (long)xcd * p.mx_per_xcd + slot / p.ny;
    if (slot / p.ny >= p.mx_per_xcd) return;
    const long m0 = (mtile * 4 + wave) * (PF * 16);
    const int nf0 = ntile * NT;
    if (m0 >= p.M) return;

    long pix_base[PF];
    int ih0[PF], iw0[PF];
#pragma unroll
    for (int pf = 0; pf < PF; ++pf) {
        long m = min(m0 + pf * 16 + pl_, p.M - 1);
        if (IS1X1) {
// ... 32 lines not shown
    auto comp = [](const float4& v, int j) { return j == 0 ? v.x : j == 1 ? v.y : j == 2 ? v.z : v.w; };

    auto chunk = [&](int kc, float4 (&xc)[PF], const bool (&okc)[PF], const float4 (&wc)[NT], float4 (&xn)[PF], bool (&okn)[PF], float4 (&wn)[NT]) {
        const int kn = min(kc + 1, p.KC - 1);
        constexpr int NM = NT * PF * 4, NL = PF + NT;
        constexpr int GAP = NM / (NL + 1) > 0 ? NM / (NL + 1) : 1;
        int cnt = 0, li = 0;
        if (!IS1X1) {
#pragma clang loop unroll(full)
            for (int pf = 0; pf < PF; ++pf) {
                float4 v = xc[pf];
                v.x = okc[pf] ? v.x : 0.f; v.y = okc[pf] ? v.y : 0.f; v.z = okc[pf] ? v.z : 0.f; v.w = okc[pf] ? v.w : 0.f;
                xc[pf] = v;
            }
        }
#pragma clang loop unroll(full)
        for (int nf = 0; nf < NT; ++nf)
#pragma clang loop unroll(full)
            for (int j = 0; j < 4; ++j)
#pragma clang loop unroll(full)
                for (int pf = 0; pf < PF; ++pf) {
                    acc[nf][pf] = __builtin_amdgcn_mfma_f32_16x16x4f32(comp(wc[nf], j), comp(xc[pf], j), acc[nf][pf], 0, 0, 0);
                    ++cnt;
                    if (cnt % GAP == 0 && li < NL) {
                        __builtin_amdgcn_sched_barrier(0);
                        if (li < PF) load_x1(kn, li, xn[li], okn[li]);
                        else load_w1(kn, li - PF, wn[li - PF]);
                        __builtin_amdgcn_sched_barrier(0);
                        ++li;
                    }
                }
    };

    float4 xa[PF], xb[PF], wa[NT], wb[NT];
    bool oka[PF], okb[PF];
#pragma clang loop unroll(full)
    for (int pf = 0; pf < PF; ++pf) load_x1(0, pf, xa[pf], oka[pf]);
#pragma clang loop unroll(full)
    for (int nf = 0; nf < NT; ++nf) load_w1(0, nf, wa[nf]);
    int kc = 0;
    for (; kc + 1 < p.KC; kc += 2) {
        chunk(kc, xa, oka, wa, xb, okb, wb);
        chunk(kc + 1, xb, okb, wb, xa, oka, wa);
    }
    if (kc < p.KC) chunk(kc, xa, oka, wa, xb, okb, wb);

    igemm_epilogue<NT, PF>(p, acc, m0, pl_, g, nf0, !bias_in_acc);
}

template <int NT, bool IS1X1, bool SE = false>
__global__ __launch_bounds__(256, 2) void conv_igemm_small_kernel(IgemmP p) {
    constexpr int D = 4;
    const int lane = threadIdx.x & 63, wave = threadIdx.x >> 6;
    const int pl_ = lane & 15, g = lane >> 4;
    const long b = blockIdx.x;
    const int ntile = (int)(b % p.ny);
    const long m0 = ((b / p.ny) * 4 + wave) * 16;
    const int nf0 = ntile * NT;
    if (m0 >= p.M) return;
    long pix_base;
    int ih0 = 0, iw0 = 0;
    {
        const long m = min(m0 + pl_, p.M - 1);
        if (IS1X1) {
            pix_base = m * (long)p.Cin;
        } else {
            const long hw = (long)p.Ho * p.Wo;
            const long n = m / hw, r = m - n * hw;
            const int oh = (int)(r / p.Wo), ow = (int)(r - (long)oh * p.Wo);
            pix_base = n * (long)p.H * p.W * p.Cin;
            ih0 = oh * p.sh - p.pt; iw0 = ow * p.sw - p.pl;
        }
    }
    f32x4 acc[NT][1];
    const bool bias_in_acc = igemm_init_acc<NT, 1>(p, acc, g, nf0);
    const float4* wf = reinterpret_cast<const float4*>(p.w) + ((long)nf0 * p.KC) * 64 + lane;

    float4 xs[D], ws[D][NT], gs[SE ? D : 1];
    bool ok[D];
    const float* se_row = SE ? p.se + (min(m0 + pl_, p.M - 1) / p.se_hw) * (long)p.K : nullptr;
    auto request = [&](int kc_, int d) {
        const int kc = min(kc_, p.KC - 1);
        const int k = min(kc * 16 + 4 * g, p.K - 4);
        if (IS1X1) {
            xs[d] = *reinterpret_cast<const float4*>(p.x + pix_base + k);
            if (SE) gs[d] = *reinterpret_cast<const float4*>(se_row + k);
            ok[d] = true;
        } else {
            const int tap = (int)__umulhi((unsigned)k, p.cin_magic), ci = k - tap * p.Cin;
            const int tap_h = igemm_tap_h(p, tap), tap_w = tap - tap_h * p.kw;
            const int ih = ih0 + tap_h * p.dh, iw = iw0 + tap_w * p.dw;
            ok[d] = ih >= 0 && ih < p.H && iw >= 0 && iw < p.W;
            const int ihc = min(max(ih, 0), p.H - 1), iwc = min(max(iw, 0), p.W - 1);
            xs[d] = *reinterpret_cast<const float4*>(p.x + pix_base + ((long)ihc * p.W + iwc) * p.Cin + ci);
        }
#pragma clang loop unroll(full)
        for (int nf = 0; nf < NT; ++nf) ws[d][nf] = wf[((long)nf * p.KC + kc) * 64];
    };
    auto comp = [](const float4& v, int j) { return j == 0 ? v.x : j == 1 ? v.y : j == 2 ? v.z : v.w; };
    auto consume = [&](int d) {
        float4 v = xs[d];
        if (!IS1X1) { v.x = ok[d] ? v.x : 0.f; v.y = ok[d] ? v.y : 0.f; v.z = ok[d] ? v.z : 0.f; v.w = ok[d] ? v.w : 0.f; }
        if (SE) { const float4 gq = gs[d]; v.x *= gq.x; v.y *= gq.y; v.z *= gq.z; v.w *= gq.w; }
#pragma clang loop unroll(full)
        for (int j = 0; j < 4; ++j)
#pragma clang loop unroll(full)
            for (int nf = 0; nf < NT; ++nf)
                acc[nf][0] = __builtin_amdgcn_mfma_f32_16x16x4f32(comp(ws[d][nf], j), comp(v, j), acc[nf][0], 0, 0, 0);
    };
#pragma clang loop unroll(full)
    for (int d = 0; d < D; ++d) request(d, d);
    int kc = 0;
    for (; kc + D <= p.KC; kc += D) {
#pragma clang loop unroll(full)
        for (int d = 0; d < D; ++d) {
            consume(d);
            request(kc + d + D, d);
        }
    }
    const int rem = p.KC - kc;
#pragma clang loop unroll(full)
    for (int d = 0; d < D - 1; ++d)
        if (d < rem) consume(d);
    igemm_epilogue<NT, 1>(p, acc, m0, pl_, g, nf0, !bias_in_acc);
}


static int ws_x6_tile(int K, int nfrag) {
    const int KC = (K + 31) / 32;
    const int cand[3] = {8, 6, 4};
    int best = 1 << 30, nt = 0;
    for (int t : cand) {
        if ((size_t)t * KC * 3072 > 150 * 1024) continue;
        int padded = (nfrag + t - 1) / t * t;
        if (padded < best) { best = padded; nt = t; }
    }
    return nt;
}

int ctc_tiles(int n_padded) { return ((n_padded + 15) / 16 + 7) / 8; }
bool ctc_partials_supported(int K) { return K % 4 == 0 && K >= 32 && (size_t)8 * ((K + 15) / 16) * 1024 <= 150 * 1024; }
bool ctc_partials_supported_x6(int K) { return K % 8 == 0 && K >= 32 && (size_t)8 * ((K + 31) / 32) * 3072 <= 150 * 1024; }

static int os_mode() { static const int m = [] { const char* e = getenv("OAR_IGEMM_OS"); return e ? atoi(e) : 1; }(); return m; }
static bool os_x6_eligible(long M, int K, int N, int Cin, bool grouped = false) {
    static const int min_k = [] { const char* e = getenv("OAR_IGEMM_OS_MINK"); return e ? atoi(e) : 256; }();
    const long tiles = ((M + 255) / 256) * ((N + 127) / 128);
    const bool fills = M >= 65536 || (M >= 8192 && tiles >= 256) || (grouped && M >= 4096) || (K >= 2048 && M >= 8192 && tiles >= 128);
    return Cin % 8 == 0 && K >= min_k && N >= (grouped ? 32 : 48) && (N & 3) == 0 && fills && K < 65536;
}

std::vector<int> conv3x3_n16_slices(long M, int Cin, int Cout, long img_px, int y_ld) { return conv3x3_n16_x6_slices(M, Cin, Cout, img_px, y_ld); }
bool conv_msrc_ok(long M, int K, int N) { return os_mode() != 0 && (K & 7) == 0 && os_x6_eligible(M, K, N, K) && igemm_weight_format(M, K, N, true, K) == IGEMM_W_X6; }
bool conv_grouped_x6_ok(long M, int K, int N, int Cin) { return os_mode() != 0 && os_x6_eligible(M, K, N, Cin, true); }

int igemm_weight_format(long M, int K, int N, bool is1x1, int Cin, long same3x3_px, bool lk_ok) {
    static const int mode = [] { const char* e = getenv("OAR_IGEMM_X6"); return e ? atoi(e) : 1; }();
    if (!mode) return IGEMM_W_K16;
    if (!is1x1 && same3x3_px > 0 && K == 9 * Cin && conv3x3_n16_x6_eligible(M, Cin, N, same3x3_px, 4 * N)) return IGEMM_W_X6;
    if (!is1x1 && lk_ok) return IGEMM_W_X6;
    if (!is1x1) return (os_mode() && Cin > 0 && os_x6_eligible(M, K, N, Cin)) ? IGEMM_W_X6 : IGEMM_W_K16;
    const int nfrag = (N + 15) / 16;
    const long passes = ((M + 15) / 16) * ((nfrag + 7) / 8);
    if (K % 8 == 0 && K >= 96 && N >= 96 && (N & 3) == 0 && passes >= 4096 && ws_x6_tile(K, nfrag) > 0) return IGEMM_W_X6;
    if (os_mode() && os_x6_eligible(M, K, N, K)) return IGEMM_W_X6;
    return IGEMM_W_K16;
}

int ws_x6_se_rows(long M, int ny, int hw);
static bool f32_1x1_goes_small(long M, int K, int N) {
    static const int ws_mode = [] { const char* e = getenv("OAR_IGEMM_WS"); return e ? atoi(e) : -1; }();
    static const int ws_min_n = [] { const char* e = getenv("OAR_IGEMM_WS_MIN_N"); return e ? atoi(e) : 96; }();
    static const long small_max = [] { const char* e = getenv("OAR_IGEMM_SMALL"); return e ? atol(e) : 4096L; }();
    const int nfrag = (N + 15) / 16, KC = (K + 15) / 16;
    int NT = 1, best = 1 << 30;
    for (int t = 4; t >= 1; --t) { int padded = (nfrag + t - 1) / t * t; if (padded < best) { best = padded; NT = t; } }
    const long ny = (nfrag + NT - 1) / NT;
    const long wave_tile_passes = ((M + 15) / 16) * ((nfrag + 7) / 8);
    const bool ws_auto = (N >= ws_min_n && wave_tile_passes >= 4096) || (K >= 512 && M >= 262144);
    const bool ws = (N & 3) == 0 && KC >= 2 && ws_mode != 0 && (ws_mode == 1 || ws_auto);
    return !ws && ((M + 15) / 16) * ny <= small_max;
}
bool conv_igemm_se_ok(long M, int K, int N, int hw) {
    static const bool on = [] { const char* e = getenv("OAR_FUSE_SE_SCALE"); return !e || atoi(e) != 0; }();
    if (!on || hw <= 0) return false;
    if (igemm_weight_format(M, K, N, true) == IGEMM_W_K16) {
        const char* e = getenv("OAR_FUSE_SE_SCALE_SMALL");
        const bool small_se = !(e && e[0] == '0');
        return small_se && (K & 3) == 0 && (N & 3) == 0 && f32_1x1_goes_small(M, K, N);
    }
    if (igemm_weight_format(M, K, N, true) != IGEMM_W_X6) return false;
    const int nfrag = (N + 15) / 16, nt = ws_x6_tile(K, nfrag);
    if (nt == 0 || os_mode() == 2) return false;
    const int ny = (nfrag + nt - 1) / nt;
    const size_t lds = (size_t)nt * ((K + 31) / 32) * 3072 + (size_t)nt * 64 + 16 + (size_t)ws_x6_se_rows(M, ny, hw) * K * 4;
    return lds <= 160 * 1024;
}

void conv_igemm(hipStream_t s, const ConvP& c) {
    IgemmP p;
    p.x = c.x; p.w = c.w; p.bias = c.bias; p.res = c.residual; p.y = c.y;
    p.H = c.H; p.W = c.W; p.Cin = c.Cin; p.kh = c.kh; p.kw = c.kw; p.sh = c.sh; p.sw = c.sw;
    p.pt = c.pt; p.pl = c.pl; p.dh = c.dh; p.dw = c.dw; p.y_ld = c.y_ld;
    p.act = c.act.kind; p.alpha = c.act.alpha; p.beta = c.act.beta;
    p.convt = c.convt2x2; p.Cout = c.Cout;
    p.ctc_part = c.ctc_part; p.ctc_valid = c.ctc_valid;
    p.se = c.se; p.se_hw = c.Ho * c.Wo;
    p.x_ld = c.x_ld > 0 ? c.x_ld : c.Cin; p.accum = c.accum;
    p.n_msrc = c.n_msrc;
    for (int i = 0; i < 8; ++i) { p.msrc[i] = i < c.n_msrc ? c.msrc[i] : nullptr; p.msrc_c[i] = i < c.n_msrc ? c.msrc_c[i] : 0; }
    p.res_up = c.residual ? c.res_up : 0;
    if (c.convt2x2) {
        p.Ho = c.H; p.Wo = c.W;
        p.M = (long)c.N * c.H * c.W; p.K = c.Cin; p.gemm_cout = 4 * c.Cout;
    } else {
        p.Ho = c.Ho; p.Wo = c.Wo;
        p.M = (long)c.N * c.Ho * c.Wo; p.K = c.kh * c.kw * c.Cin; p.gemm_cout = c.Cout;
    }
    const bool x6 = c.w_fmt == IGEMM_W_X6;
    const bool grouped = p.x_ld != c.Cin;
    p.KC = x6 ? (p.K + 31) / 32 : (p.K + 15) / 16;
    if (p.M == 0) return;
    const bool is1x1 = c.convt2x2 || (c.kh == 1 && c.kw == 1 && c.sh == 1 && c.sw == 1 && c.pt == 0 && c.pl == 0);
    int nfrag = (p.gemm_cout + 15) / 16;
    int NT = 1;
    {
        int best = 1 << 30;
        for (int t = 4; t >= 1; --t) { int padded = (nfrag + t - 1) / t * t; if (padded < best) { best = padded; NT = t; } }
    }
    const long ny = (nfrag + NT - 1) / NT;
    static const int pf_max = [] { const char* e = getenv("OAR_IGEMM_PF"); int v = e ? atoi(e) : 2; return v == 1 || v == 4 ? v : 2; }();
    int PF = pf_max;
    while (PF > 1 && ((p.M + 4L * PF * 16 - 1) / (4L * PF * 16)) * ny < 1024) PF >>= 1;
    const long mx = (p.M + 4L * PF * 16 - 1) / (4L * PF * 16);
    p.ny = (int)ny;
    OAR_CHECK(p.K < 65536, OAR_UNSUPPORTED_OP, "conv_igemm: K = kh*kw*Cin must be < 65536");
    p.cin_magic = (unsigned)((1ull << 32) / (unsigned)c.Cin + 1);
    p.kw_magic = (unsigned)((1ull << 32) / (unsigned)c.kw + 1);
    p.kw_one = c.kw == 1 ? 1u : 0u;
    p.mx_per_xcd = (mx + 7) / 8;
    dim3 grid((unsigned)(p.mx_per_xcd * 8 * ny));
    static const int ws_mode = [] { const char* e = getenv("OAR_IGEMM_WS"); return e ? atoi(e) : -1; }();
    static const int ws_min_n = [] { const char* e = getenv("OAR_IGEMM_WS_MIN_N"); return e ? atoi(e) : 96; }();
    int ws_nt = 0;
    const bool vec_ok = ((p.Cout & 3) == 0) && ((p.y_ld & 3) == 0);
    const long wave_tile_passes = ((p.M + 15) / 16) * ((nfrag + 7) / 8);
    const bool ws_auto = (p.gemm_cout >= ws_min_n && wave_tile_passes >= 4096) || (p.K >= 512 && p.M >= 262144);
    const bool res_up = p.res_up > 1;
    OAR_CHECK(!res_up || (!x6 && !c.convt2x2 && p.M < (1L << 31) && c.Ho % p.res_up == 0 && c.Wo % p.res_up == 0), OAR_INTERNAL, "conv_igemm: upsampled residual on an ineligible layer");
    if (!x6 && !res_up && vec_ok && p.KC >= 2 && ws_mode != 0 && (ws_mode == 1 || ws_auto)) {
        static const int max_nt = [] { const char* e = getenv("OAR_IGEMM_WS_MAXNT"); return e ? atoi(e) : 8; }();
        const int cand[6] = {8, 6, 4, 3, 2, 1};
        int best = 1 << 30;
        for (int t : cand) {
            if (t > max_nt || (size_t)t * p.KC * 1024 > 150 * 1024) continue;
            int padded = (nfrag + t - 1) / t * t;
            if (padded < best) { best = padded; ws_nt = t; }
        }
    }
    if (c.ctc_part && x6 && is1x1 && !c.residual && !c.se && c.act.kind == ACT_NONE && ctc_head_x6_supported(p.M, p.K, p.gemm_cout)) {
        ctc_head_x6(s, c.x, c.w, c.bias, c.ctc_part, p.M, p.K, p.gemm_cout, c.ctc_valid);
        return;
    }
    if (c.ctc_part) {
        OAR_CHECK(vec_ok && is1x1 && (x6 ? ctc_partials_supported_x6(p.K) : ctc_partials_supported(p.K)), OAR_INTERNAL, "conv_igemm: CTC partials on an ineligible layer");
        ws_nt = 8;
    }
    const bool ws3 = !x6 && !res_up && !c.ctc_part && conv_igemm_ws3_eligible(p, nfrag);
    const bool ws = ws_nt > 0 || ws3;
    static const long small_max = [] { const char* e = getenv("OAR_IGEMM_SMALL"); return e ? atol(e) : 4096L; }();
    const bool small = !x6 && !ws && ((p.M + 15) / 16) * ny <= small_max;
    double flops = 2.0 * (double)p.M * p.K * p.gemm_cout;
    double bytes = 4.0 * ((double)c.N * c.H * c.W * c.Cin + (double)p.M * p.gemm_cout + (double)p.K * p.gemm_cout);
    char pname[96];
    static const bool os_wide = [] { const char* e = getenv("OAR_IGEMM_OS_WIDE"); return !e || atoi(e) != 0; }();
    const bool cheap_act = c.act.kind == ACT_NONE || c.act.kind == ACT_RELU;
    const bool prefer_os = os_wide && os_mode() != 0 && x6 && is1x1 && !c.convt2x2 && !c.se && !c.ctc_part && cheap_act && p.K >= 320 && p.gemm_cout >= 512 && ws_x6_tile(p.K, nfrag) > 0 && ws_x6_tile(p.K, nfrag) <= 4 &&
                           os_x6_eligible(p.M, p.K, p.gemm_cout, c.Cin);
    const bool x6_os = x6 && !c.ctc_part && (!is1x1 || ws_x6_tile(p.K, nfrag) == 0 || prefer_os || c.n_msrc > 0 || (os_mode() == 2 && os_x6_eligible(p.M, p.K, p.gemm_cout, c.Cin)));
    const bool rs3_cls = x6 && !c.convt2x2 && c.kh == 3 && c.kw == 3 && c.sh == 1 && c.sw == 1 && c.pt == 1 && c.pl == 1 && c.dh == 1 && c.dw == 1 && c.Ho == c.H && c.Wo == c.W && !c.residual && !c.se &&
                         !c.ctc_part && conv3x3_n16_x6_eligible(p.M, c.Cin, c.Cout, (long)c.H * c.W, c.y_ld);
    const bool lk = x6 && !c.ctc_part && !c.se && !c.convt2x2 && !is1x1 &&
                    conv_lk_x6_eligible(c.kh, c.kw, c.sh, c.sw, c.pt, c.pl, c.dh, c.dw, c.H, c.W, c.Ho, c.Wo, c.Cin, c.Cout, c.y_ld, p.M);
    const char* cls = lk ? "conv_lk_x6" : rs3_cls ? "conv_rs3_x6" : x6_os ? "conv_igemm_os_x6" : x6 ? "conv_igemm_ws_x6" : ws ? "conv_igemm_ws" : "conv_igemm";
    if (Profiler::get().detail) {
        snprintf(pname, sizeof pname, "conv_igemm%s M=%ld K=%d N=%d k%dx%d s%d%s", lk ? "_lk_x6" : rs3_cls ? "_rs3_x6" : x6_os ? "_os_x6" : x6 ? "_x6" : ws ? "_ws" : "", p.M, p.K, p.gemm_cout, c.kh, c.kw, c.sh, c.convt2x2 ? " convT" : "");
        cls = pname;
    }
    ProfScope ps(s, cls, bytes, flops);
#define LAUNCH2(NTV, PFV)                                                                                          \
    do {                                                                                                          \
        if (is1x1) hipLaunchKernelGGL((conv_igemm_kernel<NTV, PFV, true>), grid, dim3(256), 0, s, p);     \
        else hipLaunchKernelGGL((conv_igemm_kernel<NTV, PFV, false>), grid, dim3(256), 0, s, p);                 \
    } while (0)
#define LAUNCH(NTV)                                  \
    do {                                             \
        if (PF == 4) LAUNCH2(NTV, 4);                \
        else if (PF == 2) LAUNCH2(NTV, 2);           \
        else LAUNCH2(NTV, 1);                        \
    } while (0)
    OAR_CHECK(!c.se || x6 || (small && is1x1 && !c.residual && !c.convt2x2), OAR_INTERNAL, "conv_igemm: gate on a layer neither gated kernel takes (conv_igemm_se_ok should have said no)");
    const bool same3x3 = !c.convt2x2 && c.kh == 3 && c.kw == 3 && c.sh == 1 && c.sw == 1 && c.pt == 1 && c.pl == 1 && c.dh == 1 && c.dw == 1 && c.Ho == c.H && c.Wo == c.W;
    const bool rs3 = x6 && same3x3 && !c.residual && !c.se && !c.ctc_part && conv3x3_n16_x6_eligible(p.M, c.Cin, c.Cout, (long)c.H * c.W, c.y_ld);
    OAR_CHECK(!(x6 && same3x3 && c.Cout <= 16) || rs3, OAR_INTERNAL, "conv_igemm: 3x3 / Cout <= 16 bf16x6 weights but the row-streaming kernel's launch-time conditions do not hold (y_ld / output size / residual / gate changed after planning)");
    OAR_CHECK(!grouped || (x6 && !is1x1 && !c.ctc_part && !c.se && !c.convt2x2 && (rs3 || !(same3x3 && c.Cout <= 16))), OAR_INTERNAL, "conv_igemm: x_ld on a layer that runs on neither kernel that reads x with a stride of its own");
    OAR_CHECK(c.n_msrc == 0 || (x6 && is1x1 && !c.convt2x2 && !c.ctc_part && !c.se && !lk), OAR_INTERNAL, "conv_igemm: multi-source input on a layer that does not run on the output-stationary bf16x6 kernel");
    OAR_CHECK(!c.accum || rs3, OAR_INTERNAL, "conv_igemm: accumulate flag on a layer that does not run on the row-streaming 3x3 kernel");
    if (lk) {
        conv_lk_x6(s, p, c.N);
    } else if (ws3) {
        conv_igemm_ws3(s, p, nfrag);
    } else if (rs3) {
        conv3x3_n16_x6(s, p, c.N);
    } else if (x6) {
        const int nt = c.ctc_part ? 8 : is1x1 ? ws_x6_tile(p.K, nfrag) : 0;
        OAR_CHECK(((p.Cout & 3) == 0) && ((p.y_ld & 3) == 0) && !c.convt2x2, OAR_INTERNAL, "conv_igemm: bf16x6 weights on an ineligible layer");
        const bool os = !c.ctc_part && (nt == 0 || prefer_os || c.n_msrc > 0 || (os_mode() == 2 && os_x6_eligible(p.M, p.K, p.gemm_cout, c.Cin)));
        OAR_CHECK(!c.se || (!os && !c.ctc_part && is1x1), OAR_INTERNAL, "conv_igemm: gate on a layer the weight-stationary x6 kernel does not take");
        if (os) {
            OAR_CHECK(os_x6_eligible(p.M, p.K, p.gemm_cout, c.Cin, grouped), OAR_INTERNAL, "conv_igemm: bf16x6 weights on a layer neither x6 kernel takes");
            conv_igemm_os_x6(s, p, nfrag, is1x1);
        } else {
            conv_igemm_ws_x6(s, p, nt, (nfrag + nt - 1) / nt, (size_t)nt * p.KC * 3072 + (size_t)nt * 64 + 16);
        }
    } else if (ws) {
        const int wny = (nfrag + ws_nt - 1) / ws_nt;
        const size_t lds = (size_t)ws_nt * p.KC * 1024 + (size_t)ws_nt * 64 + 16;
        if (is1x1) conv_igemm_ws_1x1(s, p, ws_nt, wny, lds);
        else conv_igemm_ws_gen(s, p, ws_nt, wny, lds);
    } else if (small) {
        const dim3 sgrid((unsigned)(((p.M + 63) / 64) * ny));
#define LAUNCH_SMALL(NTV)                                                                                          \
    do {                                                                                                          \
        if (is1x1 && p.se) hipLaunchKernelGGL((conv_igemm_small_kernel<NTV, true, true>), sgrid, dim3(256), 0, s, p); \
        else if (is1x1) hipLaunchKernelGGL((conv_igemm_small_kernel<NTV, true>), sgrid, dim3(256), 0, s, p);   \
        else hipLaunchKernelGGL((conv_igemm_small_kernel<NTV, false>), sgrid, dim3(256), 0, s, p);             \
    } while (0)
        if (NT == 4) LAUNCH_SMALL(4);
        else if (NT == 3) LAUNCH_SMALL(3);
        else if (NT == 2) LAUNCH_SMALL(2);
        else LAUNCH_SMALL(1);
#undef LAUNCH_SMALL
    } else if (NT == 4) LAUNCH(4);
    else if (NT == 3) LAUNCH(3);
    else if (NT == 2) LAUNCH(2);
    else LAUNCH(1);
#undef LAUNCH2
#undef LAUNCH
}

}
}
```

### oar_ocr_amd/csrc/igemm_dev.h

```cpp
#pragma once
#include <hip/hip_runtime.h>

#include <algorithm>
#include <cstdio>
#include <cstdlib>
#include <type_traits>
#include <vector>

#include "common.h"
#include "kernels_dev.h"

namespace oar {
namespace k {

struct IgemmP {
    const float* x;
    const float* w;
    const float* bias;
    const float* res;
    float* y;
    long M;
    int K, KC;
    int gemm_cout;
    int Cout;
    int H, W, Cin, Ho, Wo, kh, kw, sh, sw, pt, pl, dh, dw;
    int y_ld;
    int act, convt;
    int ny;
    unsigned cin_magic, kw_magic;
    unsigned kw_one;
    long mx_per_xcd;
    float alpha, beta;
    float* ctc_part;
    int ctc_valid;
    int res_up;
    const float* se;
    int se_hw;
    int n_msrc;
    const float* msrc[8];
    int msrc_c[8];
    int accum;
    int x_ld;
};

__device__ __forceinline__ int igemm_tap_h(const IgemmP& p, int tap) { return (int)(__umulhi((unsigned)tap, p.kw_magic) + (unsigned)tap * p.kw_one); }

__device__ __forceinline__ long igemm_res_off(const IgemmP& p, long opix, int co) {
    if (p.res_up <= 1) return opix * p.y_ld + co;
    const unsigned hw = (unsigned)(p.Ho * p.Wo), m = (unsigned)opix, f = (unsigned)p.res_up;
    const unsigned n = m / hw, r = m - n * hw, h = r / (unsigned)p.Wo, w = r - h * (unsigned)p.Wo;
    return (((long)n * (p.Ho / p.res_up) + h / f) * (long)(p.Wo / p.res_up) + w / f) * p.Cout + co;
}

__device__ __forceinline__ void igemm_store(const IgemmP& p, f32x4 v, bool valid, long obase, int c, bool vec_ok, bool add_bias = true) {
    if (!valid || c >= p.gemm_cout) return;
    float o[4] = {v[0], v[1], v[2], v[3]};
    if (vec_ok) {
        int co = c; long opix = obase;
        if (p.convt) { int ab = c / p.Cout; co = c - ab * p.Cout; opix = obase + (long)(ab >> 1) * (2L * p.Wo) + (ab & 1); }
        if (p.bias && add_bias) { float4 bv = *reinterpret_cast<const float4*>(p.bias + co); o[0] += bv.x; o[1] += bv.y; o[2] += bv.z; o[3] += bv.w; }
        float* dst = p.y + opix * p.y_ld + co;
        if (p.res) { float4 rv = *reinterpret_cast<const float4*>(p.res + igemm_res_off(p, opix, co)); o[0] += rv.x; o[1] += rv.y; o[2] += rv.z; o[3] += rv.w; }
#pragma unroll
        for (int r = 0; r < 4; ++r) o[r] = apply_act(o[r], p.act, p.alpha, p.beta);
        *reinterpret_cast<float4*>(dst) = make_float4(o[0], o[1], o[2], o[3]);
    } else {
#pragma unroll
        for (int r = 0; r < 4; ++r) {
            int cc = c + r;
            if (cc >= p.gemm_cout) continue;
            int co = cc; long opix = obase;
            if (p.convt) { int ab = cc / p.Cout; co = cc - ab * p.Cout; opix = obase + (long)(ab >> 1) * (2L * p.Wo) + (ab & 1); }
            float t = o[r];
            if (p.bias && add_bias) t += p.bias[co];
            if (p.res) t += p.res[igemm_res_off(p, opix, co)];
            p.y[opix * p.y_ld + co] = apply_act(t, p.act, p.alpha, p.beta);
        }
    }
}

template <int NT, int PF, bool VEC_ONLY = false>
__device__ __forceinline__ void igemm_epilogue(const IgemmP& p, f32x4 (&acc)[NT][PF], long m0, int pl_, int g, int nf0, bool add_bias) {
    const bool vec_ok = ((p.Cout & 3) == 0) && ((p.y_ld & 3) == 0);
    long obase[PF];
    bool mvalid[PF];
#pragma clang loop unroll(full)
    for (int pf = 0; pf < PF; ++pf) {
        const long m = m0 + pf * 16 + pl_;
        mvalid[pf] = m < p.M;
        const long mc = mvalid[pf] ? m : p.M - 1;
        obase[pf] = mc;
        if (p.convt) {
            long hw = (long)p.Ho * p.Wo;
            long n = mc / hw; long r = mc - n * hw;
            int h = (int)(r / p.Wo), w = (int)(r - (long)h * p.Wo);
            obase[pf] = (n * (2L * p.Ho) + 2L * h) * (2L * p.Wo) + 2L * w;
        }
    }
    if (!VEC_ONLY && !vec_ok) {
#pragma clang loop unroll(full)
        for (int pf = 0; pf < PF; ++pf)
#pragma clang loop unroll(full)
            for (int nf = 0; nf < NT; ++nf) igemm_store(p, acc[nf][pf], mvalid[pf], obase[pf], (nf0 + nf) * 16 + g * 4, false, add_bias);
        return;
    }
    auto coff = [&](int nf, int pf, bool& cvalid, int& co) -> long {
        const int c = (nf0 + nf) * 16 + g * 4;
        cvalid = c < p.gemm_cout;
        const int cc = cvalid ? c : 0;
        co = cc; long dpix = 0;
        if (p.convt) { int ab = cc / p.Cout; co = cc - ab * p.Cout; dpix = (long)(ab >> 1) * (2L * p.Wo) + (ab & 1); }
        return (obase[pf] + dpix) * p.y_ld + co;
    };
    if (p.bias && add_bias) {
        float4 bv[NT];
#pragma clang loop unroll(full)
        for (int nf = 0; nf < NT; ++nf) { bool cv; int co; (void)coff(nf, 0, cv, co); bv[nf] = *reinterpret_cast<const float4*>(p.bias + co); }
#pragma clang loop unroll(full)
        for (int nf = 0; nf < NT; ++nf)
#pragma clang loop unroll(full)
            for (int pf = 0; pf < PF; ++pf) { acc[nf][pf][0] += bv[nf].x; acc[nf][pf][1] += bv[nf].y; acc[nf][pf][2] += bv[nf].z; acc[nf][pf][3] += bv[nf].w; }
    }
    if (p.res) {
        float4 rv[NT][PF];
#pragma clang loop unroll(full)
        for (int nf = 0; nf < NT; ++nf)
#pragma clang loop unroll(full)
            for (int pf = 0; pf < PF; ++pf) {
                bool cv; int co;
                long ro = coff(nf, pf, cv, co);
                if constexpr (!VEC_ONLY) { if (p.res_up > 1) ro = igemm_res_off(p, obase[pf], co); }
                rv[nf][pf] = *reinterpret_cast<const float4*>(p.res + ro);
            }
#pragma clang loop unroll(full)
        for (int nf = 0; nf < NT; ++nf)
#pragma clang loop unroll(full)
            for (int pf = 0; pf < PF; ++pf) { acc[nf][pf][0] += rv[nf][pf].x; acc[nf][pf][1] += rv[nf][pf].y; acc[nf][pf][2] += rv[nf][pf].z; acc[nf][pf][3] += rv[nf][pf].w; }
    }
    auto act_all = [&](auto f) {
#pragma clang loop unroll(full)
        for (int nf = 0; nf < NT; ++nf)
#pragma clang loop unroll(full)
            for (int pf = 0; pf < PF; ++pf)
#pragma clang loop unroll(full)
                for (int r = 0; r < 4; ++r) acc[nf][pf][r] = f(acc[nf][pf][r]);
    };
    switch (p.act) {
        case ACT_NONE: break;
        case ACT_RELU: act_all([](float v) { return v > 0.f ? v : 0.f; }); break;
        case ACT_HSWISH: act_all([](float v) { float t = fminf(fmaxf(v * (1.0f / 6.0f) + 0.5f, 0.f), 1.f); return v * t; }); break;
        default: { const int kind = p.act; const float al = p.alpha, be = p.beta; act_all([=](float v) { return apply_act(v, kind, al, be); }); } break;
    }
#pragma clang loop unroll(full)
    for (int nf = 0; nf < NT; ++nf)
#pragma clang loop unroll(full)
        for (int pf = 0; pf < PF; ++pf) {
            bool cv; int co;
            const long o = coff(nf, pf, cv, co);
            if (mvalid[pf] && cv) *reinterpret_cast<float4*>(p.y + o) = make_float4(acc[nf][pf][0], acc[nf][pf][1], acc[nf][pf][2], acc[nf][pf][3]);
        }
}

template <int NT>
__device__ __forceinline__ void igemm_ctc_epilogue(const IgemmP& p, f32x4 (&acc)[NT][1], long m0, int pl_, int g, int nf0, int ntile, int ny) {
    float m = -3.402823466e38f;
#pragma clang loop unroll(full)
    for (int nf = 0; nf < NT; ++nf)
#pragma clang loop unroll(full)
        for (int r = 0; r < 4; ++r) {
            const int c = (nf0 + nf) * 16 + g * 4 + r;
            if (c < p.ctc_valid) m = fmaxf(m, acc[nf][0][r]);
        }
    m = fmaxf(m, __shfl_xor(m, 16, 64));
    m = fmaxf(m, __shfl_xor(m, 32, 64));
    float sum = 0.f;
    int last = -1;
#pragma clang loop unroll(full)
    for (int nf = 0; nf < NT; ++nf)
#pragma clang loop unroll(full)
        for (int r = 0; r < 4; ++r) {
            const int c = (nf0 + nf) * 16 + g * 4 + r;
            if (c < p.ctc_valid) {
                const float e = __expf(acc[nf][0][r] - m);
                sum += e;
                if (e == 1.0f) last = c;
            }
        }
    sum += __shfl_xor(sum, 16, 64);
    sum += __shfl_xor(sum, 32, 64);
    last = max(last, __shfl_xor(last, 16, 64));
    last = max(last, __shfl_xor(last, 32, 64));
    const long row = m0 + pl_;
    if (g == 0 && row < p.M) {
        float4* dst = reinterpret_cast<float4*>(p.ctc_part) + row * ny + ntile;
        *dst = make_float4(m, sum, __int_as_float(last), 0.f);
    }
}

template <int NT, int PF>
__device__ __forceinline__ bool igemm_init_acc(const IgemmP& p, f32x4 (&acc)[NT][PF], int g, int nf0) {
    const bool fast = p.bias != nullptr && ((p.Cout & 3) == 0) && ((p.y_ld & 3) == 0);
#pragma clang loop unroll(full)
    for (int nf = 0; nf < NT; ++nf) {
        float4 b = make_float4(0.f, 0.f, 0.f, 0.f);
        if (fast) {
            const int c = (nf0 + nf) * 16 + g * 4;
            const int cc = c < p.gemm_cout ? c : 0;
            const int co = p.convt ? cc % p.Cout : cc;
            b = *reinterpret_cast<const float4*>(p.bias + co);
        }
#pragma clang loop unroll(full)
        for (int pf = 0; pf < PF; ++pf) acc[nf][pf] = (f32x4){b.x, b.y, b.z, b.w};
    }
    return fast;
}

void conv_igemm_ws_1x1(hipStream_t s, const IgemmP& p, int ws_nt, int ny, size_t lds);
void conv_igemm_ws_gen(hipStream_t s, const IgemmP& p, int ws_nt, int ny, size_t lds);
void conv_igemm_ws_x6(hipStream_t s, const IgemmP& p, int ws_nt, int ny, size_t lds);
int igemm_os_x6_tile(int nfrag);
void conv_igemm_os_x6(hipStream_t s, const IgemmP& p, int nfrag, bool is1x1);
bool conv_igemm_ws3_eligible(const IgemmP& p, int nfrag);
void conv_igemm_ws3(hipStream_t s, const IgemmP& p, int nfrag);
bool conv3x3_n16_x6_eligible(long M, int Cin, int Cout, long img_px, int y_ld);
std::vector<int> conv3x3_n16_x6_slices(long M, int Cin, int Cout, long img_px, int y_ld);
void conv_lk_x6(hipStream_t s, const IgemmP& p, int n_images);
void conv3x3_n16_x6(hipStream_t s, const IgemmP& p, int n_images);

}
}
```

### oar_ocr_amd/csrc/kernels.h

```cpp
#pragma once
#include <hip/hip_runtime.h>

#include <cstdint>
#include <vector>

namespace oar {
namespace k {

enum ActKind : int { ACT_NONE = 0, ACT_RELU, ACT_HSWISH, ACT_HSIGMOID, ACT_SIGMOID, ACT_SWISH, ACT_LEAKY, ACT_CLIP, ACT_TANH, ACT_GELU_ERF,
                     ACT_ERF, ACT_SQRT, ACT_EXP, ACT_ABS, ACT_NEG, ACT_RECIP, ACT_LOG, ACT_GELU_TANH, ACT_SOFTPLUS, ACT_FLOOR, ACT_CEIL, ACT_ROUND, ACT_NOT };
struct Act {
    int kind = ACT_NONE;
    float alpha = 0.f, beta = 0.f;
};

struct ConvP {
    int N, H, W, Cin;
    int Ho, Wo, Cout;
    int kh, kw, sh, sw, pt, pl, dh, dw, groups;
    Act act;
    const float* x;
    const float* w;
    const float* bias;
    const float* residual;
    float* y;
    int y_ld;
    int convt2x2;
    int w_fmt;
    float* ctc_part;
    int ctc_valid;
    const float* se;
    int res_up;
    int n_msrc;
    const float* msrc[8];
    int msrc_c[8];
    int accum;
    int x_ld;
    float* gap_part;
};
enum : int { IGEMM_W_K16 = 0, IGEMM_W_X6 = 1, IGEMM_W_X6RS = 2, IGEMM_W_X6CS = 3 };

void conv_igemm(hipStream_t s, const ConvP& p);
int igemm_weight_format(long M, int K, int N, bool is1x1, int Cin = 0, long same3x3_px = 0, bool lk_ok = false);
bool conv_lk_x6_eligible(int kh, int kw, int sh, int sw, int pt, int pl, int dh, int dw, int H, int W, int Ho, int Wo, int Cin, int Cout, int y_ld, long M);
bool conv_grouped_x6_ok(long M, int K, int N, int Cin);
bool conv_msrc_ok(long M, int K, int N);
std::vector<int> conv3x3_n16_slices(long M, int Cin, int Cout, long img_px, int y_ld);
bool conv_igemm_se_ok(long M, int K, int N, int hw);
void conv_dw(hipStream_t s, const ConvP& p);
int conv_dw_gap_tiles(const ConvP& p);
void global_avgpool_finish(hipStream_t s, const float* part, float* y, int N, int tiles, int C, int hw);
void conv_direct(hipStream_t s, const ConvP& p);
struct StemImg { const uint8_t* ptr; int32_t w; int32_t pad; };
struct StemU8 { const uint8_t* pages[32]; int src[3]; float alpha[3], beta[3]; const StemImg* dev = nullptr; };
void conv_smallcin_u8(hipStream_t s, const ConvP& p, const StemU8& st);
struct ConvT2Pair {
    const float* x; float* y;
    const float *w1, *b1, *w2, *b2;
    int N, H, W, C0, C1, C2;
    Act act1, act2;
};
bool convt2x2_pair_supported(int C0, int C1, int C2);
void convt2x2_pair(hipStream_t s, const ConvT2Pair& p);
void convt_direct(hipStream_t s, const ConvP& p);

struct PoolP {
    int N, H, W, C, Ho, Wo, kh, kw, sh, sw, pt, pl;
    int pb, pr;
    int is_max, count_include_pad;
    const float* x;
    float* y;
};
void pool2d(hipStream_t s, const PoolP& p);
int global_avgpool_splits(int N, int HW, int C);
void global_avgpool(hipStream_t s, const float* x, float* y, int N, int HW, int C, float* partial = nullptr);

int resize_nearest_index(int o, float scale, int in, int out, int ctm, int nearest_mode);
void binary_upsampled(hipStream_t s, const float* a, const float* b, float* y, int N, int Ho, int Wo, int C, int fh, int fw, int op);
void resize(hipStream_t s, const float* x, float* y, int N, int H, int W, int C, int Ho, int Wo, float scale_h,
            float scale_w, int mode, int ctm, int nearest_mode, int y_ld);
struct ConcatGatherP { const float* x[8]; int c[8], off[8], fh[8], fw[8]; int n_src, N, Ho, Wo, C; };
void concat_gather(hipStream_t s, const ConcatGatherP& p, float* y);

void unary(hipStream_t s, const float* x, float* y, int64_t n, Act act);
void binary(hipStream_t s, const float* a, const float* b, float* y, int op, int rank, const int64_t* dims,
            const int64_t* sa, const int64_t* sb, Act post);
void copy2d(hipStream_t s, const float* x, float* y, int64_t rows, int c, int x_ld, int y_ld);
void permute(hipStream_t s, const float* x, float* y, int rank, const int64_t* out_dims, const int64_t* in_strides);

struct GemmP {
    int batch, M, N, K, transB;
    int64_t sA, sB, sC;
    float alpha;
    const float *A, *B, *bias, *residual;
    float* C;
    Act act;
};
void gemm_batched(hipStream_t s, const GemmP& p);

void layernorm(hipStream_t s, const float* x, const float* gamma, const float* beta, float* y, int64_t rows, int C, float eps);
void softmax_lastdim(hipStream_t s, const float* x, float* y, int64_t rows, int C);
void se_fc(hipStream_t s, const float* x, const float* w1, const float* b1, Act act1, const float* w2, const float* b2, Act act2, float* y, int N, int C,
           int Cmid, int Cout, int tiles = 0, int hw = 0);
void pad_nd(hipStream_t s, const float* x, float* y, int rank, const int64_t* in_dims, const int64_t* out_dims, const int64_t* before, int mode, float value);
void reduce_lastdim(hipStream_t s, const float* x, float* y, int64_t rows, int C, int mode);
void argreduce_lastdim(hipStream_t s, const float* x, float* y, int64_t rows, int C, bool is_min, bool select_last);
inline void reduce_mean_lastdim(hipStream_t s, const float* x, float* y, int64_t rows, int C) { reduce_lastdim(s, x, y, rows, C, 0); }
void where(hipStream_t s, const float* cond, const float* a, const float* b, float* y, int rank, const int64_t* dims, const int64_t* sc, const int64_t* sa, const int64_t* sb);
void grid_sample(hipStream_t s, const float* x, const float* grid, float* y, int N, int H, int W, int C, int Ho, int Wo, int mode, int padding, int align_corners);
void attention(hipStream_t s, const float* qkv, float* out, int n, int T, int heads, int hd, float scale);
bool attention_x6_supported(int T, int heads, int hd);
void attention_x6(hipStream_t s, const float* qkv, float* out, int n, int T, int heads, int hd, float scale);
bool attention_fits(int T, int heads, int hd);
enum ChainType : int { CH_GEMM = 0, CH_LN = 1, CH_ATTN = 2, CH_COPY = 3, CH_POOL = 4 };
struct ChainRef { unsigned long long v = 0; int kind = -1; };
struct ChainOpD {
    int type = 0;
    int K = 0, N = 0;
    int cin = 0, pad = 0;
    int ksplit = 1;
    int mb = 1;
    int in_ld = 0, out_ld = 0, res_ld = 0;
    int act = 0; float alpha = 0.f, beta = 0.f;
    float eps = 0.f, scale = 0.f;
    int heads = 0, hd = 0;
    ChainRef in, out, res;
    const float* w = nullptr;
    int bias_l = -1;
    int w_l = -1;
};
static_assert(sizeof(ChainOpD) % 4 == 0, "ChainOpD is copied to LDS word by word");
struct ChainLaunch {
    const ChainOpD* ops = nullptr; int n_ops = 0, n_samples = 0, T = 0, max_hd = 0;
    size_t lds = 0;
    const float* consts = nullptr; int small = 0, total_consts = 0, small_l = 0;
    int tab_l = 0;
    double bytes = 0, flops = 0;
};
constexpr size_t kChainLdsBudget = 159 * 1024;
constexpr int kChainMaxHd = 16;
inline bool chain_act_ok(int kind) { return kind == ACT_NONE || kind == ACT_RELU || kind == ACT_HSWISH || kind == ACT_HSIGMOID || kind == ACT_SIGMOID || kind == ACT_SWISH; }
size_t chain_lds_bytes(const ChainOpD& op, int T);
void chain_run(hipStream_t s, const ChainLaunch& L, char* arena, const char* input);
int ctc_tiles(int n_padded);
bool ctc_partials_supported(int K);
bool ctc_partials_supported_x6(int K);
void ctc_combine(hipStream_t s, const float* part, int64_t rows, int tiles, int64_t* idx, float* prob);
bool ctc_head_x6_supported(long M, int K, int n_padded);
void ctc_head_x6(hipStream_t s, const float* x, const float* w_x6, const float* bias, float* part, long M, int K, int n_padded, int valid);
void softmax_argmax(hipStream_t s, const float* logits, int64_t rows, int C, int ld, int64_t* idx, float* prob);

}
}
```

Baseline: 2469 images/sec.

## Fuse nearest-upsample and concat into the 3x3 row-streaming conv via multi-source gather

Adds a new 3x3 bf16x6 row-streaming conv kernel that reads its input directly from up to four separate source tensors, each optionally at a power-of-two nearest-upsample factor. The planner can now defer both the concat and any pending nearest Resize feeding a 3x3 conv, which is the typical DB neck-to-head pattern. This avoids materialising the upsampled maps and the concatenated tensor. The cost is extra address arithmetic in the load path, a larger liveness window for the pre-resize sources, and a requirement that all sources sit in the arena within a 32-bit offset span. Debug prints for concat deferral are removed and the byte estimates are updated.

```diff
diff --git a/oar_ocr_amd/build.py b/oar_ocr_amd/build.py
--- a/oar_ocr_amd/build.py
+++ b/oar_ocr_amd/build.py
@@ -10,7 +10,7 @@
 CSRC = HERE / "csrc"
 LIBDIR = HERE / "lib"
 LIB = LIBDIR / "libOarMi355x.so"
-SOURCES = ["common.cc", "onnx_parse.cc", "engine.cc", "db_host.cc", "poly_host.cc", "pipeline.cc", "c_api.cc", "ctc_host.cc", "image_decode.cc", "image_misc_decode.cc", "jpeg_decode.cc", "layout.cc", "kernels.hip", "igemm.hip", "igemm_ws_1x1.hip", "igemm_ws_gen.hip", "igemm_ws_x6.hip", "igemm_os_x6.hip", "igemm_ws3.hip", "igemm_rs3_x6.hip", "prepost.hip", "contours.hip", "jpeg.hip", "layout.hip", "dsblock.hip", "dsblock_k3s1.hip", "dsblock_k3s2.hip", "dsblock_k5s1.hip", "dsblock_k5s2.hip", "dsblock_wa_a.hip", "dsblock_wa_b.hip", "dsblock_rs_k3s11.hip", "dsblock_rs_k3s21.hip", "dsblock_rs_k3s12.hip", "dsblock_rs_k3s22.hip", "dsblock_rs_dbg.hip", "dsblock_cs.hip", "dsblock_pc.hip", "dsblock_rs2.hip", "ctc_head_x6.hip", "chain.hip", "attention_x6.hip", "igemm_lk_x6.hip"]
+SOURCES = ["common.cc", "onnx_parse.cc", "engine.cc", "db_host.cc", "poly_host.cc", "pipeline.cc", "c_api.cc", "ctc_host.cc", "image_decode.cc", "image_misc_decode.cc", "jpeg_decode.cc", "layout.cc", "kernels.hip", "igemm.hip", "igemm_ws_1x1.hip", "igemm_ws_gen.hip", "igemm_ws_x6.hip", "igemm_os_x6.hip", "igemm_ws3.hip", "igemm_rs3_x6.hip", "igemm_rs3_x6_gather.hip", "prepost.hip", "contours.hip", "jpeg.hip", "layout.hip", "dsblock.hip", "dsblock_k3s1.hip", "dsblock_k3s2.hip", "dsblock_k5s1.hip", "dsblock_k5s2.hip", "dsblock_wa_a.hip", "dsblock_wa_b.hip", "dsblock_rs_k3s11.hip", "dsblock_rs_k3s21.hip", "dsblock_rs_k3s12.hip", "dsblock_rs_k3s22.hip", "dsblock_rs_dbg.hip", "dsblock_cs.hip", "dsblock_pc.hip", "dsblock_rs2.hip", "ctc_head_x6.hip", "chain.hip", "attention_x6.hip", "igemm_lk_x6.hip"]
 HIPCC = os.environ.get("HIPCC", "/opt/rocm/bin/hipcc")
 FLAGS = ["--offload-arch=gfx950", "-O3", "-std=c++17", "-fPIC", "-ffp-contract=off", "-fno-fast-math",
          "-Wno-unused-result", "-Wno-pass-failed"]
diff --git a/oar_ocr_amd/csrc/engine.cc b/oar_ocr_amd/csrc/engine.cc
--- a/oar_ocr_amd/csrc/engine.cc
+++ b/oar_ocr_amd/csrc/engine.cc
@@ -678,20 +678,22 @@
              4.0 * ((double)q.N * q.H * q.W * q.C + (double)q.N * q.Ho * q.Wo * q.C));
     }
     std::map<std::string, const GNode*> pending_convt;
-    struct PendingConcat { std::vector<Loc> src; std::vector<int> c; std::vector<int64_t> dims; };
+    struct PendingConcat { std::vector<Loc> src; std::vector<int> c; std::vector<int> f; std::vector<int64_t> dims; };
     std::map<std::string, PendingConcat> pending_concat;
     std::map<std::string, int> concat_consumer;
     void emit_concat_gather(const PendingConcat& pc, Loc yl) {
         k::ConcatGatherP gp{};
         gp.n_src = (int)pc.src.size(); gp.N = (int)pc.dims[0]; gp.Ho = (int)pc.dims[2]; gp.Wo = (int)pc.dims[3]; gp.C = (int)pc.dims[1];
         int off = 0;
-        for (size_t i = 0; i < pc.src.size(); ++i) { gp.c[i] = pc.c[i]; gp.off[i] = off; gp.fh[i] = 1; gp.fw[i] = 1; off += pc.c[i]; }
+        for (size_t i = 0; i < pc.src.size(); ++i) { gp.c[i] = pc.c[i]; gp.off[i] = off; gp.fh[i] = gp.fw[i] = pc.f[i]; off += pc.c[i]; }
         const std::vector<Loc> src = pc.src;
+        double bytes = 4.0 * (double)numel(pc.dims);
+        for (size_t i = 0; i < pc.src.size(); ++i) bytes += 4.0 * (double)(pc.dims[0] * pc.dims[2] * pc.dims[3]) * pc.c[i] / ((double)pc.f[i] * pc.f[i]);
         step([=](const RunCtx& c) {
             k::ConcatGatherP q = gp;
             for (int i = 0; i < q.n_src; ++i) q.x[i] = c.at(src[(size_t)i]);
             k::concat_gather(c.s, q, c.mut(yl));
-        }, 0, 8.0 * (double)numel(pc.dims));
+        }, 0, bytes);
     }
     void materialise_concat(const std::string& name) {
         auto it = pending_concat.find(name);
@@ -1334,6 +1336,17 @@
         }
     }
 
+    bool conv3x3_reads_concat(const GNode& n, const std::vector<int64_t>& wd, const std::vector<int64_t>& pd) {
+        if (wd.size() != 4 || wd[2] != 3 || wd[3] != 3 || wd[1] != pd[1] || n.ai("group", 1) != 1) return false;
+        auto st = n.ais("strides"), dl = n.ais("dilations");
+        for (auto e : st) if (e != 1) return false;
+        for (auto e : dl) if (e != 1) return false;
+        int64_t pt, pl, pb, pr;
+        get_pads(n, pd[2], pd[3], 3, 3, 1, 1, 1, 1, pt, pl, pb, pr);
+        if (pt != 1 || pl != 1 || pb != 1 || pr != 1) return false;
+        return k::conv3x3_msrc_ok((long)(pd[0] * pd[2] * pd[3]), (int)pd[1], (int)wd[0], (long)(pd[2] * pd[3]));
+    }
+
     void op_conv(const GNode& n) {
         if (n.in.size() > 3 && !n.in[3].empty()) {
             TInfo xg = get(n.in[0]), gt = get(n.in[3]);
@@ -1361,10 +1374,11 @@
             if (pit != pending_concat.end()) {
                 auto wi = E.inits_.find(n.in.size() > 1 ? n.in[1] : std::string());
                 const std::vector<int64_t>& pd = pit->second.dims;
-                const bool still_ok = wi != E.inits_.end() && wi->second.dims.size() == 4 && wi->second.dims[2] == 1 && wi->second.dims[3] == 1 && n.residual.empty() &&
-                                      !(n.in.size() > 3 && !n.in[3].empty()) && n.out.size() == 1 &&
-                                      k::conv_msrc_ok((long)(pd[0] * pd[2] * pd[3]), (int)pd[1], (int)wi->second.dims[0]);
-                if (getenv("OAR_DEBUG_CONCAT")) fprintf(stderr, "  conv %s reads pending concat: still_ok=%d (w4=%d res=%d gate=%d nout=%zu)\n", n.out[0].c_str(), (int)still_ok, (int)(wi != E.inits_.end() && wi->second.dims.size() == 4), (int)!n.residual.empty(), (int)(n.in.size() > 3 && !n.in[3].empty()), n.out.size());
+                bool still_ok = wi != E.inits_.end() && wi->second.dims.size() == 4 && n.residual.empty() && !(n.in.size() > 3 && !n.in[3].empty()) && n.out.size() == 1;
+                bool up = false;
+                for (int f : pit->second.f) up = up || f != 1;
+                if (still_ok && wi->second.dims[2] == 1 && wi->second.dims[3] == 1) still_ok = !up && k::conv_msrc_ok((long)(pd[0] * pd[2] * pd[3]), (int)pd[1], (int)wi->second.dims[0]);
+                else still_ok = still_ok && conv3x3_reads_concat(n, wi->second.dims, pd);
                 if (still_ok) { msrc = pit->second; TInfo keep = vals[n.in[0]]; pending_concat.erase(pit); vals[n.in[0]] = keep; }
             }
         }
@@ -1526,12 +1540,16 @@
         }
         const bool from_concat = !msrc.src.empty();
         OAR_CHECK(!from_concat || (kind == 0 && p.w_fmt == k::IGEMM_W_X6), OAR_INTERNAL, "Conv: deferred concat in front of a layer that is not on the bf16x6 kernels");
+        if (from_concat) {
+            bytes = 4.0 * (N * Ho * Wo * Cout + numel(W.dims));
+            for (size_t i = 0; i < msrc.src.size(); ++i) bytes += 4.0 * (double)(N * H * Wd) * msrc.c[i] / ((double)msrc.f[i] * msrc.f[i]);
+        }
         auto run = [=](const RunCtx& c) {
             k::ConvP q = p;
             q.y = c.mut(yl); q.residual = has_res ? c.at(res) : nullptr; q.se = has_gate ? c.at(gate) : nullptr;
             if (from_concat) {
                 q.x = nullptr; q.n_msrc = (int)msrc.src.size();
-                for (int i = 0; i < q.n_msrc; ++i) { q.msrc[i] = c.at(msrc.src[(size_t)i]); q.msrc_c[i] = msrc.c[(size_t)i]; }
+                for (int i = 0; i < q.n_msrc; ++i) { q.msrc[i] = c.at(msrc.src[(size_t)i]); q.msrc_c[i] = msrc.c[(size_t)i]; q.msrc_f[i] = msrc.f[(size_t)i]; }
             } else {
                 q.x = c.at(xin);
             }
@@ -2529,8 +2547,8 @@
             int64_t coff = 0, total = pod[pax] * inner;
             bool plain = !absorb && r == 4 && inner == 1 && xs.size() >= 3 && (od[1] & 3) == 0;
             for (auto& t : xs) plain = plain && t.dims.size() == 4 && (t.dims[1] & 3) == 0;
-            static const bool defer_on = [] { const char* e = getenv("OAR_CONCAT_DEFER"); return !(e && e[0] == '0'); }();
-            if (getenv("OAR_DEBUG_CONCAT")) fprintf(stderr, "concat %s: plain=%d absorb=%d r=%d inner=%ld n=%zu consumer=%d\n", n.out[0].c_str(), (int)plain, (int)absorb, r, (long)inner, xs.size(), concat_consumer.count(n.out[0]) ? concat_consumer[n.out[0]] : -1);
+            const char* defer_env = getenv("OAR_CONCAT_DEFER");
+            const bool defer_on = !(defer_env && defer_env[0] == '0');
             if (plain && defer_on && xs.size() <= 8 && concat_consumer.count(n.out[0])) {
                 const GNode& cn = E.nodes_[concat_consumer[n.out[0]]];
                 auto wi = E.inits_.find(cn.in.size() > 1 ? cn.in[1] : std::string());
@@ -2539,14 +2557,46 @@
                           attr_ok("strides", 1) && attr_ok("pads", 0) && attr_ok("dilations", 1) && cn.residual.empty() && !(cn.in.size() > 3 && !cn.in[3].empty()) &&
                           cn.as("auto_pad", "NOTSET") == "NOTSET";
                 for (auto& t : xs) ok = ok && t.layout == Layout::CLAST && (t.dims[1] & 7) == 0 && t.dims[0] == od[0] && t.dims[2] == od[2] && t.dims[3] == od[3] && !t.host_int;
-                if (getenv("OAR_DEBUG_CONCAT")) {
-                    fprintf(stderr, "  ok before msrc check = %d (K=%ld N=%ld) res=%d gate=%d autopad=%s\n", (int)ok, (long)od[1], wi != E.inits_.end() ? (long)wi->second.dims[0] : -1L, (int)!cn.residual.empty(), (int)(cn.in.size() > 3 && !cn.in[3].empty()), cn.as("auto_pad", "NOTSET").c_str());
-                    for (auto& t : xs) fprintf(stderr, "    src layout=%d C=%ld host=%d\n", (int)(t.layout == Layout::CLAST), (long)t.dims[1], (int)t.host_int);
-                }
                 ok = ok && k::conv_msrc_ok((long)(od[0] * od[2] * od[3]), (int)od[1], (int)wi->second.dims[0]) && (wi->second.dims[0] & 3) == 0;
                 if (ok) {
                     PendingConcat pc;
-                    for (size_t i = 0; i < xs.size(); ++i) { pc.src.push_back(ins[i]); pc.c.push_back((int)xs[i].dims[1]); }
+                    for (size_t i = 0; i < xs.size(); ++i) { pc.src.push_back(ins[i]); pc.c.push_back((int)xs[i].dims[1]); pc.f.push_back(1); }
+                    pc.dims = od;
+                    TInfo t;
+                    t.dims = od; t.layout = Layout::CLAST;
+                    vals[n.out[0]] = t;
+                    pending_concat[n.out[0]] = std::move(pc);
+                    return;
+                }
+            }
+            if ((absorb || plain) && defer_on && r == 4 && inner == 1 && (int)xs.size() <= k::conv3x3_msrc_max() && concat_consumer.count(n.out[0])) {
+                const GNode& cn = E.nodes_[concat_consumer[n.out[0]]];
+                auto wi = E.inits_.find(cn.in.size() > 1 ? cn.in[1] : std::string());
+                bool ok = wi != E.inits_.end() && cn.residual.empty() && !(cn.in.size() > 3 && !cn.in[3].empty()) && cn.out.size() == 1 && conv3x3_reads_concat(cn, wi->second.dims, od);
+                PendingConcat pc;
+                size_t lo = ~(size_t)0, hi = 0;
+                for (size_t i = 0; ok && i < xs.size(); ++i) {
+                    const PendingResize* pr = peek_pending(n.in[i]);
+                    const TInfo& t = xs[i];
+                    ok = t.dims.size() == 4 && (t.dims[1] & 3) == 0 && t.dims[0] == od[0] && t.dims[2] == od[2] && t.dims[3] == od[3] && !t.host_int;
+                    Loc l;
+                    int f = 1;
+                    if (pr) {
+                        f = pr->fh;
+                        ok = ok && f > 0 && pr->fw == f && (f & (f - 1)) == 0 && f <= 16 && pr->imode == 0 && pr->N == od[0] && pr->C == t.dims[1] && pr->H * f == od[2] && pr->W * f == od[3];
+                        l = pr->xin;
+                    } else {
+                        ok = ok && t.layout == Layout::CLAST;
+                        l = ins[i];
+                    }
+                    ok = ok && l.kind == Loc::ARENA;
+                    if (!ok) break;
+                    const size_t b = (size_t)numel(t.dims) * 4 / ((size_t)f * f);
+                    lo = std::min(lo, (size_t)l.off); hi = std::max(hi, (size_t)l.off + b);
+                    pc.src.push_back(l); pc.c.push_back((int)t.dims[1]); pc.f.push_back(f);
+                }
+                if (ok && hi - lo < ((size_t)15 << 28)) {
+                    for (auto& nm : n.in) pending_resize.erase(nm);
                     pc.dims = od;
                     TInfo t;
                     t.dims = od; t.layout = Layout::CLAST;
@@ -3076,6 +3126,11 @@
                 if (cn.op != "Conv" || cn.in.empty() || cn.in[0] != n.out[0]) continue;
                 concat_consumer[n.out[0]] = u->second.second;
                 for (auto& sname : n.in) { int& l = lu[sname]; l = std::max(l, u->second.second); }
+                for (auto& sname : n.in) {
+                    if (!sole_consumer.count(sname)) continue;
+                    for (const GNode& rn : E.nodes_)
+                        if (rn.op == "Resize" && !rn.out.empty() && rn.out[0] == sname && !rn.in.empty()) { int& l = lu[rn.in[0]]; l = std::max(l, u->second.second); }
+                }
             }
         }
         for (int i = (int)E.nodes_.size() - 1; i >= 0; --i) {
diff --git a/oar_ocr_amd/csrc/igemm.hip b/oar_ocr_amd/csrc/igemm.hip
--- a/oar_ocr_amd/csrc/igemm.hip
+++ b/oar_ocr_amd/csrc/igemm.hip
@@ -208,6 +208,8 @@
 
 std::vector<int> conv3x3_n16_slices(long M, int Cin, int Cout, long img_px, int y_ld) { return conv3x3_n16_x6_slices(M, Cin, Cout, img_px, y_ld); }
 bool conv_msrc_ok(long M, int K, int N) { return os_mode() != 0 && (K & 7) == 0 && os_x6_eligible(M, K, N, K) && igemm_weight_format(M, K, N, true, K) == IGEMM_W_X6; }
+int conv3x3_msrc_max() { return kRs3GatherMaxSrc; }
+bool conv3x3_msrc_ok(long M, int Cin, int Cout, long img_px) { return conv3x3_n16_gather_eligible(M, Cin, Cout, img_px) && igemm_weight_format(M, 9 * Cin, Cout, false, Cin, img_px) == IGEMM_W_X6; }
 bool conv_grouped_x6_ok(long M, int K, int N, int Cin) { return os_mode() != 0 && os_x6_eligible(M, K, N, Cin, true); }
 
 int igemm_weight_format(long M, int K, int N, bool is1x1, int Cin, long same3x3_px, bool lk_ok) {
@@ -264,7 +266,7 @@
     p.se = c.se; p.se_hw = c.Ho * c.Wo;
     p.x_ld = c.x_ld > 0 ? c.x_ld : c.Cin; p.accum = c.accum;
     p.n_msrc = c.n_msrc;
-    for (int i = 0; i < 8; ++i) { p.msrc[i] = i < c.n_msrc ? c.msrc[i] : nullptr; p.msrc_c[i] = i < c.n_msrc ? c.msrc_c[i] : 0; }
+    for (int i = 0; i < 8; ++i) { p.msrc[i] = i < c.n_msrc ? c.msrc[i] : nullptr; p.msrc_c[i] = i < c.n_msrc ? c.msrc_c[i] : 0; p.msrc_f[i] = i < c.n_msrc ? c.msrc_f[i] : 0; }
     p.res_up = c.residual ? c.res_up : 0;
     if (c.convt2x2) {
         p.Ho = c.H; p.Wo = c.W;
@@ -328,6 +330,10 @@
     const bool small = !x6 && !ws && ((p.M + 15) / 16) * ny <= small_max;
     double flops = 2.0 * (double)p.M * p.K * p.gemm_cout;
     double bytes = 4.0 * ((double)c.N * c.H * c.W * c.Cin + (double)p.M * p.gemm_cout + (double)p.K * p.gemm_cout);
+    if (c.n_msrc > 0 && !is1x1) {
+        bytes = 4.0 * ((double)p.M * p.gemm_cout + (double)p.K * p.gemm_cout);
+        for (int i = 0; i < c.n_msrc; ++i) bytes += 4.0 * (double)c.N * (c.H / c.msrc_f[i]) * (c.W / c.msrc_f[i]) * c.msrc_c[i];
+    }
     char pname[96];
     static const bool os_wide = [] { const char* e = getenv("OAR_IGEMM_OS_WIDE"); return !e || atoi(e) != 0; }();
     const bool cheap_act = c.act.kind == ACT_NONE || c.act.kind == ACT_RELU;
@@ -360,12 +366,15 @@
     const bool rs3 = x6 && same3x3 && !c.residual && !c.se && !c.ctc_part && conv3x3_n16_x6_eligible(p.M, c.Cin, c.Cout, (long)c.H * c.W, c.y_ld);
     OAR_CHECK(!(x6 && same3x3 && c.Cout <= 16) || rs3, OAR_INTERNAL, "conv_igemm: 3x3 / Cout <= 16 bf16x6 weights but the row-streaming kernel's launch-time conditions do not hold (y_ld / output size / residual / gate changed after planning)");
     OAR_CHECK(!grouped || (x6 && !is1x1 && !c.ctc_part && !c.se && !c.convt2x2 && (rs3 || !(same3x3 && c.Cout <= 16))), OAR_INTERNAL, "conv_igemm: x_ld on a layer that runs on neither kernel that reads x with a stride of its own");
-    OAR_CHECK(c.n_msrc == 0 || (x6 && is1x1 && !c.convt2x2 && !c.ctc_part && !c.se && !lk), OAR_INTERNAL, "conv_igemm: multi-source input on a layer that does not run on the output-stationary bf16x6 kernel");
+    OAR_CHECK(c.n_msrc == 0 || (x6 && is1x1 && !c.convt2x2 && !c.ctc_part && !c.se && !lk) || (rs3 && !lk && !ws3 && !grouped && !c.accum), OAR_INTERNAL,
+              "conv_igemm: multi-source input on a layer that runs on neither the output-stationary bf16x6 kernel nor the row-streaming 3x3 kernel");
     OAR_CHECK(!c.accum || rs3, OAR_INTERNAL, "conv_igemm: accumulate flag on a layer that does not run on the row-streaming 3x3 kernel");
     if (lk) {
         conv_lk_x6(s, p, c.N);
     } else if (ws3) {
         conv_igemm_ws3(s, p, nfrag);
+    } else if (rs3 && c.n_msrc > 0) {
+        conv3x3_n16_gather(s, p, c.N);
     } else if (rs3) {
         conv3x3_n16_x6(s, p, c.N);
     } else if (x6) {
diff --git a/oar_ocr_amd/csrc/igemm_dev.h b/oar_ocr_amd/csrc/igemm_dev.h
--- a/oar_ocr_amd/csrc/igemm_dev.h
+++ b/oar_ocr_amd/csrc/igemm_dev.h
@@ -39,6 +39,7 @@
     int n_msrc;
     const float* msrc[8];
     int msrc_c[8];
+    int msrc_f[8];
     int accum;
     int x_ld;
 };
@@ -226,6 +227,9 @@
 std::vector<int> conv3x3_n16_x6_slices(long M, int Cin, int Cout, long img_px, int y_ld);
 void conv_lk_x6(hipStream_t s, const IgemmP& p, int n_images);
 void conv3x3_n16_x6(hipStream_t s, const IgemmP& p, int n_images);
-
-}
-}
+constexpr int kRs3GatherMaxSrc = 4;
+bool conv3x3_n16_gather_eligible(long M, int Cin, int Cout, long img_px);
+void conv3x3_n16_gather(hipStream_t s, const IgemmP& p, int n_images);
+
+}
+}
diff --git a/oar_ocr_amd/csrc/igemm_rs3_x6_gather.hip b/oar_ocr_amd/csrc/igemm_rs3_x6_gather.hip
--- /dev/null
+++ b/oar_ocr_amd/csrc/igemm_rs3_x6_gather.hip
@@ -0,0 +1,226 @@
+#include <hip/hip_ext.h>
+
+#include "igemm_dev.h"
+
+namespace oar {
+namespace k {
+
+typedef unsigned r3g_u32x4 __attribute__((ext_vector_type(4)));
+typedef unsigned r3g_u32x2 __attribute__((ext_vector_type(2)));
+typedef __bf16 r3g_bf16x8 __attribute__((ext_vector_type(8)));
+
+struct Rs3GP {
+    const float* base; float* y; const float4* w; const float* bias;
+    int N, H, W, Cin, Cout, y_ld;
+    int act; float alpha, beta;
+    int R, segs, tiles_x, items, per_xcd;
+    unsigned span, y_bytes;
+    int n_src;
+    unsigned off[kRs3GatherMaxSrc];
+    unsigned img_b[kRs3GatherMaxSrc];
+    unsigned row_sh[kRs3GatherMaxSrc];
+    unsigned c_c0[kRs3GatherMaxSrc];
+};
+
+namespace {
+constexpr unsigned kR3gOob = 0xF0000000u, kR3gOobSt = 0x80000000u;
+constexpr int kR3gIW = 18, kR3gPxB = 144, kR3gPlB = kR3gIW * kR3gPxB, kR3gRowB = 3 * kR3gPlB, kR3gWaves = 6;
+
+__device__ __forceinline__ r3g_u32x4 r3g_lds4(unsigned off) {
+    return *reinterpret_cast<const __attribute__((address_space(3))) r3g_u32x4*>((__attribute__((address_space(3))) const char*)nullptr + off);
+}
+__device__ __forceinline__ void r3g_lds_w2(unsigned off, r3g_u32x2 v) {
+    *reinterpret_cast<__attribute__((address_space(3))) r3g_u32x2*>((__attribute__((address_space(3))) char*)nullptr + off) = v;
+}
+
+template <int CC32>
+__global__ __launch_bounds__(kR3gWaves * 64, 2) void conv3x3_n16_gather_kernel(Rs3GP p) {
+    constexpr int QPP = CC32 * 8;
+    constexpr int NU = kR3gIW * QPP;
+    constexpr int NJ = (NU + 63) / 64;
+    constexpr int KC = 9 * CC32;
+    extern __shared__ float4 r3g_lds[];
+    const int tid = threadIdx.x, lane = tid & 63;
+    const int wave = __builtin_amdgcn_readfirstlane(tid >> 6);
+    const int g = lane >> 4, n = lane & 15;
+    const unsigned ring0 = (unsigned)(wave * 3 * kR3gRowB);
+
+    r3g_u32x4 wreg[KC][2];
+#pragma unroll
+    for (int kc = 0; kc < KC; ++kc)
+#pragma unroll
+        for (int s = 0; s < 2; ++s) {
+            const float4 v = p.w[(kc * 3 + s) * 64 + lane];
+            wreg[kc][s] = (r3g_u32x4){__float_as_uint(v.x), __float_as_uint(v.y), __float_as_uint(v.z), __float_as_uint(v.w)};
+        }
+    constexpr unsigned kWl = (unsigned)(kR3gWaves * 3 * kR3gRowB);
+    for (int i = tid; i < KC * 64; i += kR3gWaves * 64) r3g_lds[(kWl >> 4) + i] = p.w[((i >> 6) * 3 + 2) * 64 + (i & 63)];
+    __syncthreads();
+    const float4 bq = (p.bias && g * 4 < p.Cout) ? *reinterpret_cast<const float4*>(p.bias + g * 4) : make_float4(0.f, 0.f, 0.f, 0.f);
+
+    const int xcd = (int)(blockIdx.x & 7), wgx = (int)(blockIdx.x >> 3), wgs = (int)(gridDim.x >> 3);
+    const int b0 = xcd * p.per_xcd, b1 = min(p.items, b0 + p.per_xcd);
+    const int J = wgs * kR3gWaves, j0 = wgx * kR3gWaves + wave;
+    const int orow_bytes = p.W * p.y_ld * 4;
+    const __amdgpu_buffer_rsrc_t ysrc = __builtin_amdgcn_make_buffer_rsrc(p.y, 0, (int)p.y_bytes, 0x00020000);
+    float* const xbase = const_cast<float*>(p.base);
+    const unsigned rd_lane = (unsigned)(n * kR3gPxB + g * 16);
+
+    for (int item = b0 + j0; item < b1; item += J) {
+        const int tx = item % p.tiles_x, q_ = item / p.tiles_x, seg = q_ % p.segs, img = q_ / p.segs;
+        const int o_begin = seg * p.R, o_end = min(p.H, o_begin + p.R);
+        const int x0 = tx * 16 - 1;
+        unsigned src[NJ], rsh[NJ], dst[NJ];
+#pragma unroll
+        for (int u = 0; u < NJ; ++u) {
+            const int q = u * 64 + lane, px = q / QPP, cq = q - px * QPP, ch = cq * 4;
+            unsigned so = p.off[0] + (unsigned)img * p.img_b[0], rw = p.row_sh[0], cc = p.c_c0[0];
+#pragma unroll
+            for (int i = 1; i < kRs3GatherMaxSrc; ++i) {
+                const bool hit = i < p.n_src && ch >= (int)(p.c_c0[i] >> 16);
+                so = hit ? p.off[i] + (unsigned)img * p.img_b[i] : so;
+                rw = hit ? p.row_sh[i] : rw;
+                cc = hit ? p.c_c0[i] : cc;
+            }
+            const int xx = x0 + px, cs = (int)(cc & 0xFFFFu), c0 = (int)(cc >> 16);
+            const bool ok = q < NU && (unsigned)xx < (unsigned)p.W;
+            src[u] = ok ? so + (unsigned)((((xx >> (rw & 15u)) * cs) + (ch - c0)) * 4) : kR3gOob;
+            rsh[u] = rw;
+            dst[u] = q < NU ? (unsigned)(px * kR3gPxB + cq * 8) : 0xFFFFFFFFu;
+        }
+        r3g_u32x4 in[NJ];
+        auto load_row = [&](int y, r3g_u32x4 (&in)[NJ]) __attribute__((always_inline)) {
+            const bool rok = (unsigned)y < (unsigned)p.H;
+            const __amdgpu_buffer_rsrc_t rs = __builtin_amdgcn_make_buffer_rsrc(xbase, 0, rok ? (int)p.span : 0, 0x00020000);
+            const unsigned yy = rok ? (unsigned)y : 0u;
+#pragma unroll
+            for (int u = 0; u < NJ; ++u) {
+                const unsigned o = src[u] == kR3gOob ? kR3gOob : src[u] + (yy >> (rsh[u] & 15u)) * (rsh[u] & ~15u);
+                in[u] = __builtin_amdgcn_raw_buffer_load_b128(rs, (int)o, 0, 0);
+            }
+        };
+        auto put_row = [&](unsigned slot, const r3g_u32x4 (&in)[NJ]) __attribute__((always_inline)) {
+#pragma unroll
+            for (int u = 0; u < NJ; ++u) {
+                unsigned hb[4], mb[4], lb[4];
+#pragma unroll
+                for (int e = 0; e < 4; ++e) {
+                    const unsigned ux = in[u][e];
+                    const float xf = __uint_as_float(ux);
+                    const float r1 = xf - __uint_as_float(ux & 0xFFFF0000u);
+                    const unsigned u1 = __float_as_uint(r1);
+                    const float r2 = r1 - __uint_as_float(u1 & 0xFFFF0000u);
+                    hb[e] = ux; mb[e] = u1; lb[e] = __float_as_uint(r2);
+                }
+                if (dst[u] != 0xFFFFFFFFu) {
+                    const unsigned a = slot + dst[u];
+                    r3g_lds_w2(a, (r3g_u32x2){__builtin_amdgcn_perm(hb[1], hb[0], 0x07060302u), __builtin_amdgcn_perm(hb[3], hb[2], 0x07060302u)});
+                    r3g_lds_w2(a + kR3gPlB, (r3g_u32x2){__builtin_amdgcn_perm(mb[1], mb[0], 0x07060302u), __builtin_amdgcn_perm(mb[3], mb[2], 0x07060302u)});
+                    r3g_lds_w2(a + 2 * kR3gPlB, (r3g_u32x2){__builtin_amdgcn_perm(lb[1], lb[0], 0x07060302u), __builtin_amdgcn_perm(lb[3], lb[2], 0x07060302u)});
+                }
+            }
+        };
+        {
+            r3g_u32x4 in1[NJ], in2[NJ];
+            load_row(o_begin - 1, in);
+            load_row(o_begin, in1);
+            load_row(o_begin + 1, in2);
+            put_row(ring0, in);
+            put_row(ring0 + (unsigned)kR3gRowB, in1);
+            put_row(ring0 + (unsigned)(2 * kR3gRowB), in2);
+        }
+        int s0 = 0;
+        const int ox = tx * 16 + n;
+        const unsigned st_lane = (ox < p.W && g * 4 < p.Cout) ? (unsigned)((ox * p.y_ld + g * 4) * 4) : kR3gOobSt;
+        unsigned st_row = (unsigned)((img * p.H + o_begin) * orow_bytes);
+#pragma unroll 1
+        for (int r = o_begin; r < o_end; ++r) {
+            load_row(r + 2, in);
+            f32x4 acc[6];
+            acc[5] = (f32x4){bq.x, bq.y, bq.z, bq.w};
+            acc[0] = acc[1] = acc[2] = acc[3] = acc[4] = (f32x4){0.f, 0.f, 0.f, 0.f};
+            unsigned rd = ring0 + rd_lane;
+            unsigned slot_of[3];
+#pragma unroll
+            for (int kh = 0; kh < 3; ++kh) slot_of[kh] = (unsigned)((s0 + kh >= 3 ? s0 + kh - 3 : s0 + kh) * kR3gRowB);
+            r3g_u32x4 xs[3][4];
+            auto fetch = [&](int kc, r3g_u32x4 (&dstv)[4]) __attribute__((always_inline)) {
+                const int kh = kc / (3 * CC32), kw = (kc / CC32) % 3, c = kc % CC32;
+#pragma unroll
+                for (int s_ = 0; s_ < 3; ++s_) dstv[s_] = r3g_lds4(rd + slot_of[kh] + (unsigned)(s_ * kR3gPlB + kw * kR3gPxB + c * 64));
+                dstv[3] = r3g_lds4(rd - rd_lane - ring0 + kWl + (unsigned)(kc * 1024 + lane * 16));
+            };
+            fetch(0, xs[0]);
+            fetch(1, xs[1]);
+#pragma unroll
+            for (int kc = 0; kc < KC; ++kc) {
+                if (kc + 2 < KC) fetch(kc + 2, xs[(kc + 2) % 3]);
+                constexpr int WPL[6] = {1, 2, 0, 1, 0, 0}, XPL[6] = {1, 0, 2, 0, 1, 0};
+#pragma unroll
+                for (int t = 0; t < 6; ++t)
+                    acc[t] = __builtin_amdgcn_mfma_f32_16x16x32_bf16(__builtin_bit_cast(r3g_bf16x8, WPL[t] == 2 ? xs[kc % 3][3] : wreg[kc][WPL[t] == 2 ? 0 : WPL[t]]), __builtin_bit_cast(r3g_bf16x8, xs[kc % 3][XPL[t]]), acc[t], 0, 0, 0);
+                asm("" : "+v"(rd) : "v"(xs[kc % 3][2]));
+            }
+            f32x4 o = ((((acc[0] + acc[1]) + acc[2]) + acc[3]) + acc[4]) + acc[5];
+            r3g_u32x4 v;
+#pragma unroll
+            for (int e = 0; e < 4; ++e) v[e] = __float_as_uint(apply_act(o[e] + 0.f, p.act, p.alpha, p.beta));
+            asm volatile("s_waitcnt lgkmcnt(0)" ::: "memory");
+            put_row(ring0 + (unsigned)(s0 * kR3gRowB), in);
+            __builtin_amdgcn_raw_buffer_store_b128(v, ysrc, (int)(st_lane + st_row), 0, 0);
+            st_row += (unsigned)orow_bytes;
+            s0 = s0 + 1 == 3 ? 0 : s0 + 1;
+        }
+    }
+}
+}
+
+bool conv3x3_n16_gather_eligible(long M, int Cin, int Cout, long img_px) { return conv3x3_n16_x6_eligible(M, Cin, Cout, img_px, Cout); }
+
+void conv3x3_n16_gather(hipStream_t s, const IgemmP& g, int n_images) {
+    OAR_CHECK(g.n_msrc >= 2 && g.n_msrc <= kRs3GatherMaxSrc && !g.accum && g.x_ld == g.Cin, OAR_INTERNAL, "conv3x3_n16_gather: needs 2 ... 4 sources and a plain single-pass layer");
+    Rs3GP p{};
+    p.y = g.y; p.w = reinterpret_cast<const float4*>(g.w); p.bias = g.bias;
+    p.N = n_images; p.H = g.H; p.W = g.W; p.Cin = g.Cin; p.Cout = g.Cout; p.y_ld = g.y_ld;
+    p.act = g.act; p.alpha = g.alpha; p.beta = g.beta;
+    p.tiles_x = (g.W + 15) / 16;
+    uintptr_t lo = UINTPTR_MAX, hi = 0;
+    int csum = 0;
+    for (int i = 0; i < g.n_msrc; ++i) {
+        const int f = g.msrc_f[i], c = g.msrc_c[i];
+        int sh = 0;
+        while ((1 << sh) < f) ++sh;
+        OAR_CHECK(f >= 1 && (1 << sh) == f && sh <= 8 && c > 0 && (c & 3) == 0 && g.H % f == 0 && g.W % f == 0 && g.msrc[i] != nullptr, OAR_INTERNAL,
+                  "conv3x3_n16_gather: a source needs a power-of-two factor that divides the map and a multiple of 4 channels");
+        const size_t row_b = (size_t)(g.W / f) * c * 4, img_b = row_b * (size_t)(g.H / f);
+        const uintptr_t a = reinterpret_cast<uintptr_t>(g.msrc[i]);
+        OAR_CHECK((a & 15) == 0 && img_b * (size_t)n_images < ((size_t)1 << 32), OAR_INTERNAL, "conv3x3_n16_gather: unaligned or oversized source");
+        lo = std::min(lo, a); hi = std::max(hi, a + img_b * (size_t)n_images);
+        p.img_b[i] = (unsigned)img_b; p.row_sh[i] = (unsigned)row_b | (unsigned)sh; p.c_c0[i] = (unsigned)c | ((unsigned)csum << 16);
+        csum += c;
+    }
+    OAR_CHECK(csum == g.Cin && hi - lo < (uintptr_t)kR3gOob, OAR_INTERNAL, "conv3x3_n16_gather: the sources' channels do not add up to Cin, or they lie more than 3.75 GB apart");
+    for (int i = 0; i < g.n_msrc; ++i) p.off[i] = (unsigned)(reinterpret_cast<uintptr_t>(g.msrc[i]) - lo);
+    p.base = reinterpret_cast<const float*>(lo); p.span = (unsigned)(hi - lo); p.n_src = g.n_msrc;
+    const long waves = 256L * kR3gWaves;
+    double best = 1e30;
+    for (int R = std::min(g.H, 4); R <= g.H; ++R) {
+        const int segs = (g.H + R - 1) / R;
+        const long items = (long)n_images * segs * p.tiles_x;
+        const long rounds = (items + waves - 1) / waves;
+        const double cost = (double)rounds * (R + 2.5);
+        if (cost < best - 1e-9) { best = cost; p.R = R; p.segs = segs; p.items = (int)items; }
+    }
+    p.per_xcd = (p.items + 7) / 8;
+    p.y_bytes = (unsigned)((long)n_images * g.H * g.W * g.y_ld * 4);
+    const size_t lds = (size_t)kR3gWaves * 3 * kR3gRowB + (size_t)9 * (g.Cin / 32) * 1024;
+    auto launch = [&](auto kernel) {
+        OAR_MAX_LDS_ONCE(kernel, 160 * 1024);
+        hipLaunchKernelGGL(kernel, dim3(256), dim3(kR3gWaves * 64), lds, s, p);
+    };
+    if (g.Cin == 64) launch(conv3x3_n16_gather_kernel<2>);
+    else launch(conv3x3_n16_gather_kernel<1>);
+}
+
+}
+}
diff --git a/oar_ocr_amd/csrc/kernels.h b/oar_ocr_amd/csrc/kernels.h
--- a/oar_ocr_amd/csrc/kernels.h
+++ b/oar_ocr_amd/csrc/kernels.h
@@ -34,6 +34,7 @@
     int n_msrc;
     const float* msrc[8];
     int msrc_c[8];
+    int msrc_f[8];
     int accum;
     int x_ld;
     float* gap_part;
@@ -45,6 +46,8 @@
 bool conv_lk_x6_eligible(int kh, int kw, int sh, int sw, int pt, int pl, int dh, int dw, int H, int W, int Ho, int Wo, int Cin, int Cout, int y_ld, long M);
 bool conv_grouped_x6_ok(long M, int K, int N, int Cin);
 bool conv_msrc_ok(long M, int K, int N);
+bool conv3x3_msrc_ok(long M, int Cin, int Cout, long img_px);
+int conv3x3_msrc_max();
 std::vector<int> conv3x3_n16_slices(long M, int Cin, int Cout, long img_px, int y_ld);
 bool conv_igemm_se_ok(long M, int K, int N, int hw);
 void conv_dw(hipStream_t s, const ConvP& p);
```

Result: no change. 2470 images/sec, median of 5 (+0.1%).
